# zheminzhou/PEPPAN

Hardware: AMD Instinct MI355X
Metric: gene_pairs_aligned_per_s (higher is better)
Workload: dtype int16; 1 GPU; synthgenes-v1 seed 355: 10000 genes x 1002 nt, all-vs-all (BASELINE configs[2] search stage), min_id 0.45 min_ratio...; queries_per_rank=10000, reference_genes_per_rank=10000

## Files before the change

### peppan_amd/csrc/capi.hip

```cpp
#include "common.h"
#include <chrono>
#include <time.h>
#include <algorithm>
#include <cmath>
#include <cstring>
#include <new>

int pep_fail(pep_ctx *ctx, int code, const std::string &msg)
{
    if (ctx) { ctx->n_down = 0; ctx->pin_down_used = 0; }
    if (ctx) {
        ctx->err = msg;
        ctx->n_pending = 0;
        ctx->pin_small_used = 0;
        for (auto &st : ctx->fused_state) st.dirty = true;
        for (auto &st : ctx->scan_state) st.dirty = true;
        ctx->sort_dirty = true;
        ctx->zero_clean = false;
        for (bool &f : ctx->zero_ok) f = false;
        ctx->set_clean_slots = 0;
    }
    return code;
}

int dev_reserve(pep_ctx *ctx, DevBuf &b, size_t bytes)
{
    if (bytes <= b.cap && b.p) return PEP_OK;
    if (b.p) { (void)hipFree(b.p); b.p = nullptr; b.cap = 0; }
    size_t want = std::max<size_t>(bytes + bytes / 4, 256);
    want = (want + 255) & ~(size_t)255;
    hipError_t e = hipMalloc(&b.p, want);
    if (e != hipSuccess) {
        b.p = nullptr;
        return pep_fail(ctx, PEP_ERR_HIP, std::string("hipMalloc(") + std::to_string(want) + "): " + hipGetErrorString(e));
    }
    b.cap = want;
    return PEP_OK;
}

void dev_release(DevBuf &b)
{
    if (b.p) (void)hipFree(b.p);
    b.p = nullptr;
    b.cap = 0;
}

int pin_reserve(pep_ctx *ctx, PinBuf &b, size_t bytes)
{
    if (bytes <= b.cap) return PEP_OK;
    if (b.p) (void)hipHostFree(b.p);
    b.p = nullptr; b.cap = 0;
    const size_t want = bytes + bytes / 4 + 4096;
    PEP_HIP(ctx, hipHostMalloc(reinterpret_cast<void **>(&b.p), want, hipHostMallocDefault));
    b.cap = want;
    return PEP_OK;
}

int pep_h2d(pep_ctx *ctx, void *d_dst, const void *h_src, size_t n)
{
    if (n == 0) return PEP_OK;
    if (n < ((size_t)64 << 10) || n > ((size_t)256 << 20)) {
        PEP_HIP(ctx, hipMemcpyAsync(d_dst, h_src, n, hipMemcpyHostToDevice, ctx->stream));
        return PEP_OK;
    }
    const size_t need = (n + 255) & ~(size_t)255;
    if (ctx->pin_up_used + need > ctx->pin_up.cap) {
        if (ctx->up_event_set) { PEP_HIP(ctx, pep_event_wait(ctx->up_event)); ctx->up_event_set = false; }
        ctx->pin_up_used = 0;
        if (need > ctx->pin_up.cap) PEP_TRY(pin_reserve(ctx, ctx->pin_up, std::max(need, (size_t)32 << 20)));
    }
    memcpy(ctx->pin_up.p + ctx->pin_up_used, h_src, n);
    PEP_HIP(ctx, hipMemcpyAsync(d_dst, ctx->pin_up.p + ctx->pin_up_used, n, hipMemcpyHostToDevice, ctx->stream));
    ctx->pin_up_used += need;
    if (!ctx->up_event && hipEventCreateWithFlags(&ctx->up_event, pep_wait_event_flags()) != hipSuccess) return pep_fail(ctx, PEP_ERR_HIP, "hipEventCreate failed");
    PEP_HIP(ctx, hipEventRecord(ctx->up_event, ctx->stream));
    ctx->up_event_set = true;
    return PEP_OK;
}

int pep_d2h_queue(pep_ctx *ctx, void *h_dst, const void *d_src, size_t n)
{
    if (n == 0) return PEP_OK;
    const size_t need = (n + 255) & ~(size_t)255;
    if (n < ((size_t)64 << 10) || n > ((size_t)256 << 20) || ctx->n_down >= 16) {
        PEP_HIP(ctx, hipMemcpyAsync(h_dst, d_src, n, hipMemcpyDeviceToHost, ctx->stream));
        return PEP_OK;
    }
    if (ctx->pin_down_used + need > ctx->pin_down.cap) {
        if (ctx->n_down) {
            PEP_HIP(ctx, hipMemcpyAsync(h_dst, d_src, n, hipMemcpyDeviceToHost, ctx->stream));
            return PEP_OK;
        }
        PEP_HIP(ctx, pep_stream_wait(ctx));
        PEP_TRY(pin_reserve(ctx, ctx->pin_down, std::max(need, (size_t)16 << 20)));
        ctx->pin_down_used = 0;
    }
    PEP_HIP(ctx, hipMemcpyAsync(ctx->pin_down.p + ctx->pin_down_used, d_src, n, hipMemcpyDeviceToHost, ctx->stream));
    ctx->down[ctx->n_down++] = pep_ctx::PendingDown{h_dst, ctx->pin_down_used, n};
    ctx->pin_down_used += need;
    return PEP_OK;
}

void pep_d2h_finish(pep_ctx *ctx)
{
    for (int k = 0; k < ctx->n_down; ++k) memcpy(ctx->down[k].dst, ctx->pin_down.p + ctx->down[k].off, ctx->down[k].n);
    ctx->n_down = 0;
    ctx->pin_down_used = 0;
}

void pep_timer_begin(pep_ctx *ctx, int id)
{
    if (ctx->timing_level < (id == TM_SW ? 1 : 2)) return;
    if (!ctx->tm_a[id] && (hipEventCreate(&ctx->tm_a[id]) != hipSuccess || hipEventCreate(&ctx->tm_b[id]) != hipSuccess)) { ctx->tm_a[id] = nullptr; return; }
    ctx->tm_state[id] = hipEventRecord(ctx->tm_a[id], ctx->stream) == hipSuccess ? 1 : 0;
}

void pep_timer_end(pep_ctx *ctx, int id)
{
    if (ctx->tm_state[id] == 1) ctx->tm_state[id] = hipEventRecord(ctx->tm_b[id], ctx->stream) == hipSuccess ? 2 : 0;
}

void pep_timers_resolve(pep_ctx *ctx)
{
    double match[4] = {0., 0., 0., 0.};
    double *dst[TM_COUNT] = {&ctx->stats.ms_seed, &ctx->stats.ms_total, &ctx->stats.ms_sw, &ctx->stats.ms_sw_trace, &ctx->stats.ms_trace,
                             &match[0], &match[1], &match[2], &match[3]};
    for (int id = 0; id < TM_COUNT; ++id) {
        float ms = 0.f;
        if (ctx->tm_state[id] == 2 && hipEventSynchronize(ctx->tm_b[id]) == hipSuccess && hipEventElapsedTime(&ms, ctx->tm_a[id], ctx->tm_b[id]) == hipSuccess) *dst[id] = ms;
        ctx->tm_state[id] = 0;
    }
    ctx->stats.ms_seed_match = match[0] + match[1] + match[2] + match[3];
}

int pep_zero_block(pep_ctx *ctx, int which, size_t offset, size_t bytes, void **out)
{
    PEP_TRY(dev_reserve(ctx, ctx->d_zero, PEP_ZERO_TOTAL));
    char *p = ctx->d_zero.as<char>() + offset;
    if (!ctx->zero_ok[which]) PEP_HIP(ctx, hipMemsetAsync(p, 0, bytes, ctx->stream));
    ctx->zero_ok[which] = false;
    *out = p;
    return PEP_OK;
}

int pep_read_back(pep_ctx *ctx, void *dst, const void *d_src, size_t n)
{
    const size_t n8 = (n + 7) & ~size_t(7);
    if (ctx->n_pending >= 32 || ctx->pin_small_used + n8 > ctx->pin_small.cap) PEP_TRY(pep_sync_reads(ctx));
    if (n8 > ctx->pin_small.cap) return pep_fail(ctx, PEP_ERR_INTERNAL, "pep_read_back: value larger than the pinned page");
    PEP_HIP(ctx, hipMemcpyAsync(ctx->pin_small.p + ctx->pin_small_used, d_src, n, hipMemcpyDeviceToHost, ctx->stream));
    ctx->pending[ctx->n_pending++] = pep_ctx::PendingRead{dst, ctx->pin_small_used, n};
    ctx->pin_small_used += n8;
    return PEP_OK;
}

int pep_read_back_with_upload(pep_ctx *ctx, void *dst, const void *d_src, size_t n, void *d_up_dst, const void *pinned_up_src, uint64_t n_up_words)
{
    const size_t n8 = (n + 7) & ~size_t(7);
    if (n % 4) return pep_fail(ctx, PEP_ERR_INTERNAL, "pep_read_back_with_upload: size not a multiple of 4");
    if (ctx->n_pending >= 32 || ctx->pin_small_used + n8 > ctx->pin_small.cap) PEP_TRY(pep_sync_reads(ctx));
    if (n8 > ctx->pin_small.cap) return pep_fail(ctx, PEP_ERR_INTERNAL, "pep_read_back: value larger than the pinned page");
    PEP_TRY(pep_exchange_pinned(ctx, d_up_dst, pinned_up_src, n_up_words, ctx->pin_small.p + ctx->pin_small_used, d_src, n / 4));
    ctx->pending[ctx->n_pending++] = pep_ctx::PendingRead{dst, ctx->pin_small_used, n};
    ctx->pin_small_used += n8;
    return PEP_OK;
}

static long pep_spin_us()
{
    static const long spin_us = [] { const char *e = getenv("PEPPAN_HIP_SPIN_US"); return e ? atol(e) : 1500L; }();
    return spin_us;
}

unsigned pep_wait_event_flags() { return hipEventDisableTiming; }

hipError_t pep_event_wait(hipEvent_t ev)
{
    const long spin_us = pep_spin_us();
    if (spin_us <= 0) {
        const auto t0 = std::chrono::steady_clock::now();
        do {
            for (int spin = 0; spin < 32; ++spin) {
                const hipError_t q = hipEventQuery(ev);
                if (q != hipErrorNotReady) return q;
                __builtin_ia32_pause();
            }
        } while (std::chrono::steady_clock::now() - t0 < std::chrono::microseconds(60));
        long nap_ns = 20000;
        for (;;) {
            const hipError_t q = hipEventQuery(ev);
            if (q != hipErrorNotReady) return q;
            struct timespec ts = {0, nap_ns};
            nanosleep(&ts, nullptr);
            if (nap_ns < 200000) nap_ns += nap_ns / 2;
        }
    }
    const auto t0 = std::chrono::steady_clock::now();
    for (;;) {
        for (int spin = 0; spin < 64; ++spin) {
            const hipError_t q = hipEventQuery(ev);
            if (q != hipErrorNotReady) return q;
            __builtin_ia32_pause();
        }
        if (std::chrono::steady_clock::now() - t0 > std::chrono::microseconds(spin_us)) break;
    }
    return hipEventSynchronize(ev);
}

hipError_t pep_stream_wait(pep_ctx *ctx)
{
    if (!ctx->wait_event && hipEventCreateWithFlags(&ctx->wait_event, pep_wait_event_flags()) != hipSuccess) return hipStreamSynchronize(ctx->stream);
    const hipError_t r = hipEventRecord(ctx->wait_event, ctx->stream);
    if (r != hipSuccess) return hipStreamSynchronize(ctx->stream);
    return pep_event_wait(ctx->wait_event);
}

int pep_sync_reads(pep_ctx *ctx)
{
    const hipError_t e = pep_stream_wait(ctx);
    if (e == hipSuccess)
        for (int i = 0; i < ctx->n_pending; ++i) memcpy(ctx->pending[i].dst, ctx->pin_small.p + ctx->pending[i].off, ctx->pending[i].n);
    ctx->n_pending = 0;
    ctx->pin_small_used = 0;
    if (e != hipSuccess) return pep_fail(ctx, PEP_ERR_HIP, std::string("hipStreamSynchronize: ") + hipGetErrorString(e));
    return PEP_OK;
}

void pep_drop_dev_result(pep_ctx *ctx)
{
    pep_result *r = ctx->dev_result;
    ctx->dev_result = nullptr;
    if (r && ctx->staged_result != r) r->ctx = nullptr;
}

void pep_materialise_staged(pep_ctx *ctx)
{
    pep_result *r = ctx->staged_result;
    if (!r) return;
    r->hits.assign(r->st_hits, r->st_hits + r->n_hits);
    r->cigar.assign(r->st_cigar, r->st_cigar + r->n_cigar);
    r->st_hits = nullptr; r->st_cigar = nullptr;
    if (ctx->dev_result != r) r->ctx = nullptr;
    ctx->staged_result = nullptr;
}

int pep_upload_blk2seq(pep_ctx *ctx, SeqSet &s)
{
    const uint64_t nblk = s.total / 32 + 2;
    std::vector<uint2> m(nblk, make_uint2(0u, 0u));
    for (uint32_t i = 0; i < s.n; ++i) {
        if (s.h_len[i] == 0) continue;
        const uint64_t b0 = s.h_off[i] / 32, b1 = ((uint64_t)s.h_off[i] + s.h_len[i] - 1) / 32;
        for (uint64_t b = b0; b <= b1 && b < nblk; ++b) m[b] = make_uint2(i, s.h_off[i]);
    }
    PEP_TRY(dev_reserve(ctx, s.blk2seq, nblk * sizeof(uint2)));
    PEP_HIP(ctx, hipMemcpy(s.blk2seq.p, m.data(), nblk * sizeof(uint2), hipMemcpyHostToDevice));
    return PEP_OK;
}

namespace {

const char *kBlosum62Text =
    "   A  R  N  D  C  Q  E  G  H  I  L  K  M  F  P  S  T  W  Y  V  B  Z  X  *\n"
    "A  4 -1 -2 -2  0 -1 -1  0 -2 -1 -1 -1 -1 -2 -1  1  0 -3 -2  0 -2 -1  0 -4\n"
    "R -1  5  0 -2 -3  1  0 -2  0 -3 -2  2 -1 -3 -2 -1 -1 -3 -2 -3 -1  0 -1 -4\n"
    "N -2  0  6  1 -3  0  0  0  1 -3 -3  0 -2 -3 -2  1  0 -4 -2 -3  3  0 -1 -4\n"
    "D -2 -2  1  6 -3  0  2 -1 -1 -3 -4 -1 -3 -3 -1  0 -1 -4 -3 -3  4  1 -1 -4\n"
    "C  0 -3 -3 -3  9 -3 -4 -3 -3 -1 -1 -3 -1 -2 -3 -1 -1 -2 -2 -1 -3 -3 -2 -4\n"
    "Q -1  1  0  0 -3  5  2 -2  0 -3 -2  1  0 -3 -1  0 -1 -2 -1 -2  0  3 -1 -4\n"
    "E -1  0  0  2 -4  2  5 -2  0 -3 -3  1 -2 -3 -1  0 -1 -3 -2 -2  1  4 -1 -4\n"
    "G  0 -2  0 -1 -3 -2 -2  6 -2 -4 -4 -2 -3 -3 -2  0 -2 -2 -3 -3 -1 -2 -1 -4\n"
    "H -2  0  1 -1 -3  0  0 -2  8 -3 -3 -1 -2 -1 -2 -1 -2 -2  2 -3  0  0 -1 -4\n"
    "I -1 -3 -3 -3 -1 -3 -3 -4 -3  4  2 -3  1  0 -3 -2 -1 -3 -1  3 -3 -3 -1 -4\n"
    "L -1 -2 -3 -4 -1 -2 -3 -4 -3  2  4 -2  2  0 -3 -2 -1 -2 -1  1 -4 -3 -1 -4\n"
    "K -1  2  0 -1 -3  1  1 -2 -1 -3 -2  5 -1 -3 -1  0 -1 -3 -2 -2  0  1 -1 -4\n"
    "M -1 -1 -2 -3 -1  0 -2 -3 -2  1  2 -1  5  0 -2 -1 -1 -1 -1  1 -3 -1 -1 -4\n"
    "F -2 -3 -3 -3 -2 -3 -3 -3 -1  0  0 -3  0  6 -4 -2 -2  1  3 -1 -3 -3 -1 -4\n"
    "P -1 -2 -2 -1 -3 -1 -1 -2 -2 -3 -3 -1 -2 -4  7 -1 -1 -4 -3 -2 -2 -1 -2 -4\n"
    "S  1 -1  1  0 -1  0  0  0 -1 -2 -2  0 -1 -2 -1  4  1 -3 -2 -2  0  0  0 -4\n"
    "T  0 -1  0 -1 -1 -1 -1 -2 -2 -1 -1 -1 -1 -2 -1  1  5 -2 -2  0 -1 -1  0 -4\n"
    "W -3 -3 -4 -4 -2 -2 -3 -2 -2 -3 -2 -3 -1  1 -4 -3 -2 11  2 -3 -4 -3 -2 -4\n"
    "Y -2 -2 -2 -3 -2 -1 -2 -3  2 -1 -1 -2 -1  3 -3 -2 -2  2  7 -1 -3 -2 -1 -4\n"
    "V  0 -3 -3 -3 -1 -2 -2 -3 -3  3  1 -2  1 -1 -2 -2  0 -3 -1  4 -3 -2 -1 -4\n"
    "B -2 -1  3  4 -3  0  1 -1  0 -3 -4  0 -3 -3 -2  0 -1 -4 -3 -3  4  1 -1 -4\n"
    "Z -1  0  0  1 -3  3  4 -2  0 -3 -3  1 -1 -3 -1  0 -1 -3 -2 -2  1  4 -1 -4\n"
    "X  0 -1 -1 -1 -2 -1 -1 -1 -1 -1 -1 -1 -1 -1 -2  0  0 -2 -1 -1 -1 -1 -1 -4\n"
    "* -4 -4 -4 -4 -4 -4 -4 -4 -4 -4 -4 -4 -4 -4 -4 -4 -4 -4 -4 -4 -4 -4 -4  1\n";

void parse_blosum(int8_t sub[1024])
{
    char cols[32];
    int ncol = 0;
    const char *p = kBlosum62Text;
    while (*p != '\n') { if (*p != ' ') cols[ncol++] = *p; ++p; }
    ++p;
    int m[26][26];
    bool have[26] = {false};
    for (int r = 0; r < ncol; ++r) {
        while (*p == ' ') ++p;
        const char row = *p++;
        for (int c = 0; c < ncol; ++c) {
            char *end;
            const long v = strtol(p, &end, 10);
            p = end;
            if (row >= 'A' && row <= 'Z' && cols[c] >= 'A' && cols[c] <= 'Z') { m[row - 'A'][cols[c] - 'A'] = (int)v; have[row - 'A'] = true; }
        }
        while (*p && *p != '\n') ++p;
        if (*p) ++p;
    }
    const int X = 'X' - 'A';
    for (int a = 0; a < 32; ++a)
        for (int b = 0; b < 32; ++b) {
            int v = -64;
            if (a < 26 && b < 26) v = m[have[a] ? a : X][have[b] ? b : X];
            sub[a * 32 + b] = (int8_t)v;
        }
}

int upload_sub_image(pep_ctx *ctx)
{
    std::vector<uint32_t> img(256 * PEP_TAB_REP);
    const int8_t *s = ctx->params.sub;
    for (int w = 0; w < 256; ++w) {
        const int q = w >> 3, t0 = (w & 7) * 4;
        uint32_t v = 0;
        for (int k = 0; k < 4; ++k) v |= (uint32_t)(uint8_t)s[q * 32 + t0 + k] << (8 * k);
        for (int b = 0; b < PEP_TAB_REP; ++b) img[w * PEP_TAB_REP + b] = v;
    }
    PEP_TRY(dev_reserve(ctx, ctx->sub_lds, img.size() * 4));
    PEP_HIP(ctx, hipMemcpy(ctx->sub_lds.p, img.data(), img.size() * 4, hipMemcpyHostToDevice));
    return PEP_OK;
}

int upload_nt(pep_ctx *ctx, NtSet &s, const uint8_t *nt, const uint64_t *off, uint32_t n)
{
    if (n && (!nt || !off)) return pep_fail(ctx, PEP_ERR_ARG, "null sequence buffer");
    s.n = n;
    s.h_off.assign(n + 1, 0);
    for (uint32_t i = 0; i <= n; ++i) {
        s.h_off[i] = n ? off[i] : 0;
        if (i && s.h_off[i] < s.h_off[i - 1]) return pep_fail(ctx, PEP_ERR_ARG, "offsets must be non-decreasing");
        if (i && s.h_off[i] - s.h_off[i - 1] > 0x7FFFFF00ull) return pep_fail(ctx, PEP_ERR_LIMIT, "nucleotide sequence longer than 2^31 - 256");
    }
    s.total = s.h_off[n];
    PEP_TRY(dev_reserve(ctx, s.nt, s.total + 64));
    PEP_TRY(dev_reserve(ctx, s.off, (size_t)(n + 1) * 8));
    if (s.total) PEP_TRY(pep_h2d(ctx, s.nt.p, nt, s.total));
    PEP_TRY(pep_h2d(ctx, s.off.p, s.h_off.data(), (size_t)(n + 1) * 8));
    return PEP_OK;
}

int upload_aa(pep_ctx *ctx, SeqSet &s, const uint8_t *codes, const uint64_t *off, uint32_t n, uint32_t max_n)
{
    if (n && (!codes || !off)) return pep_fail(ctx, PEP_ERR_ARG, "null sequence buffer");
    if (n > max_n) return pep_fail(ctx, PEP_ERR_LIMIT, "too many sequences");
    if (&s == &ctx->t) ctx->t_tables_lazy = false;
    if (&s == &ctx->q) ctx->q_tables_lazy = false;
    s.n = n;
    s.h_off.assign(n + 1, 0);
    s.h_len.assign(n, 0);
    uint64_t pos = PEP_END_PAD, residues = 0;
    uint32_t max_len = 0;
    for (uint32_t i = 0; i < n; ++i) {
        if (off[i + 1] < off[i]) return pep_fail(ctx, PEP_ERR_ARG, "offsets must be non-decreasing");
        const uint64_t len = off[i + 1] - off[i];
        if (len > PEP_MAX_SEQ_LEN) return pep_fail(ctx, PEP_ERR_LIMIT, "sequence longer than PEP_MAX_SEQ_LEN");
        s.h_off[i] = (uint32_t)pos;
        s.h_len[i] = (uint32_t)len;
        residues += len;
        max_len = std::max<uint32_t>(max_len, (uint32_t)len);
        pos += (len + 15) / 16 * 16 + PEP_SEQ_GAP;
        if (pos > PEP_MAX_RESIDUES) return pep_fail(ctx, PEP_ERR_LIMIT, "packed protein set exceeds 2^29 bytes");
    }
    pos += PEP_END_PAD;
    s.h_off[n] = (uint32_t)pos;
    s.total = pos; s.residues = residues; s.max_len = max_len;
    std::vector<uint8_t> img(pos, (uint8_t)PEP_PAD_CODE);
    for (uint32_t i = 0; i < n; ++i)
        for (uint32_t x = 0; x < s.h_len[i]; ++x) {
            const uint8_t c = codes[off[i] + x];
            img[s.h_off[i] + x] = c < 26 ? c : (uint8_t)23;
        }
    PEP_TRY(dev_reserve(ctx, s.res, pos + 64));
    PEP_TRY(dev_reserve(ctx, s.off, (size_t)(n + 1) * 4));
    PEP_TRY(dev_reserve(ctx, s.len, (size_t)(n + 1) * 4));
    PEP_HIP(ctx, hipMemcpy(s.res.p, img.data(), pos, hipMemcpyHostToDevice));
    PEP_HIP(ctx, hipMemcpy(s.off.p, s.h_off.data(), (size_t)(n + 1) * 4, hipMemcpyHostToDevice));
    if (n) PEP_HIP(ctx, hipMemcpy(s.len.p, s.h_len.data(), (size_t)n * 4, hipMemcpyHostToDevice));
    return pep_upload_blk2seq(ctx, s);
}

int download_aa(pep_ctx *ctx, const SeqSet &s, uint8_t *codes, uint64_t cap, uint64_t *off)
{
    if (s.residues > cap) return pep_fail(ctx, PEP_ERR_ARG, "output buffer too small");
    PEP_TRY(pep_k1_host_tables(ctx));
    std::vector<uint8_t> img(s.total);
    if (s.total) PEP_HIP(ctx, hipMemcpy(img.data(), s.res.p, s.total, hipMemcpyDeviceToHost));
    uint64_t pos = 0;
    for (uint32_t i = 0; i < s.n; ++i) {
        off[i] = pos;
        memcpy(codes + pos, img.data() + s.h_off[i], s.h_len[i]);
        pos += s.h_len[i];
    }
    off[s.n] = pos;
    return PEP_OK;
}

}

int pep_upload_codes(pep_ctx *ctx, SeqSet &s, const uint8_t *codes, const uint64_t *off, uint32_t n, uint32_t max_n) { return upload_aa(ctx, s, codes, off, n, max_n); }
int pep_upload_sub(pep_ctx *ctx) { return upload_sub_image(ctx); }

extern "C" {

int pep_version(void) { return PEP_ABI_VERSION; }

int pep_device_count(void)
{
    int n = 0;
    if (hipGetDeviceCount(&n) != hipSuccess) return 0;
    return n;
}

void pep_default_params(pep_search_params *p)
{
    memset(p, 0, sizeof(*p));
    p->gap_open = 11; p->gap_ext = 1;
    parse_blosum(p->sub);
    memset(p->reduce, 0xFF, sizeof(p->reduce));
    const char *groups = "KREDQN/C/G/H/ILV/M/F/Y/W/P/STA";
    int g = 0;
    for (const char *c = groups; *c; ++c) { if (*c == '/') ++g; else p->reduce[*c - 'A'] = (uint8_t)g; }
    p->base = g + 1;
    const char *shapes[2] = {"111101110111", "111011010010111"};
    p->n_shapes = 2;
    for (int s = 0; s < 2; ++s) {
        int w = 0;
        for (int k = 0; shapes[s][k]; ++k) if (shapes[s][k] == '1') p->offs[s][w++] = k;
        p->weight[s] = w;
    }
    p->min_id_pct = 0.; p->min_qcov_pct = 0.; p->top_k = 10; p->n_splits = 5;
    p->dbsize = 5e6; p->max_evalue = 1.;
    p->use_lds = 1;
    p->ungapped_min = 55; p->xdrop = 12; p->ext_right = 40; p->ext_left = 24; p->stage1_min = 24; p->reserved2 = 0;
    p->ka_lambda = 0.267; p->ka_k = 0.041;
}

int pep_set_sensitivity(pep_search_params *p, int level)
{
    if (!p || level < 0 || level > 1) return PEP_ERR_ARG;
    const char *shapes[4] = {"111101110111", "111011010010111", "110010011111011", "10111110011011"};
    p->n_shapes = level == 0 ? 2 : 4;
    for (int s = 0; s < 4; ++s) {
        int w = 0;
        for (int k = 0; k < 32; ++k) p->offs[s][k] = 0;
        if (s < p->n_shapes) for (int k = 0; shapes[s][k]; ++k) if (shapes[s][k] == '1') p->offs[s][w++] = k;
        p->weight[s] = w;
    }
    return PEP_OK;
}

int32_t pep_min_score_ka(uint32_t qlen, double dbsize, double max_evalue, double ka_lambda, double ka_k)
{
    const double s = log(ka_k * (double)qlen * dbsize / max_evalue) / ka_lambda;
    const int32_t r = (int32_t)ceil(s);
    return r < 1 ? 1 : r;
}

int32_t pep_min_score(uint32_t qlen, double dbsize, double max_evalue)
{
    return pep_min_score_ka(qlen, dbsize, max_evalue, 0.267, 0.041);
}

int pep_ctx_create(int device, pep_ctx **out)
{
    if (!out) return PEP_ERR_ARG;
    *out = nullptr;
    int n = 0;
    if (hipGetDeviceCount(&n) != hipSuccess || device < 0 || device >= n) return PEP_ERR_HIP;
    pep_ctx *ctx = new (std::nothrow) pep_ctx();
    if (!ctx) return PEP_ERR_INTERNAL;
    ctx->device = device;
    memset(&ctx->stats, 0, sizeof(ctx->stats));
    pep_default_params(&ctx->params);
    if (hipSetDevice(device) != hipSuccess) { delete ctx; return PEP_ERR_HIP; }
    if (hipStreamCreate(&ctx->stream) != hipSuccess) { delete ctx; return PEP_ERR_HIP; }
    if (pin_reserve(ctx, ctx->pin_small, 16384) != PEP_OK) { *out = ctx; return PEP_ERR_HIP; }
    int rc = pep_selftest_dpp(ctx);
    if (rc != PEP_OK) { *out = ctx; return rc; }
    *out = ctx;
    return PEP_OK;
}

void pep_ctx_destroy(pep_ctx *ctx)
{
    if (!ctx) return;
    (void)hipSetDevice(ctx->device);
    for (auto &b : ctx->ws) dev_release(b);
    for (int id = 0; id < TM_COUNT; ++id) { if (ctx->tm_a[id]) (void)hipEventDestroy(ctx->tm_a[id]); if (ctx->tm_b[id]) (void)hipEventDestroy(ctx->tm_b[id]); }
    pep_drop_dev_result(ctx);
    if (ctx->staged_result) {
        pep_materialise_staged(ctx);
    }
    if (ctx->pin_small.p) (void)hipHostFree(ctx->pin_small.p);
    if (ctx->pin_stage.p) (void)hipHostFree(ctx->pin_stage.p);
    if (ctx->pin_k1.p) (void)hipHostFree(ctx->pin_k1.p);
    if (ctx->pin_k1q.p) (void)hipHostFree(ctx->pin_k1q.p);
    if (ctx->pin_labels.p) (void)hipHostFree(ctx->pin_labels.p);
    if (ctx->pin_nt_match.p) (void)hipHostFree(ctx->pin_nt_match.p);
    if (ctx->k1_event) (void)hipEventDestroy(ctx->k1_event);
    if (ctx->k1q_event) (void)hipEventDestroy(ctx->k1q_event);
    if (ctx->k1_t0) (void)hipEventDestroy(ctx->k1_t0);
    if (ctx->k1_t1) (void)hipEventDestroy(ctx->k1_t1);
    if (ctx->wait_event) (void)hipEventDestroy(ctx->wait_event);
    if (ctx->up_event) (void)hipEventDestroy(ctx->up_event);
    if (ctx->pin_down.p) (void)hipHostFree(ctx->pin_down.p);
    if (ctx->pin_up.p) (void)hipHostFree(ctx->pin_up.p);
    if (ctx->pin_ms.p) (void)hipHostFree(ctx->pin_ms.p);
    DevBuf *bufs[] = {&ctx->sub_lds, &ctx->d_params, &ctx->scan_state[0].buf, &ctx->scan_state[1].buf, &ctx->fused_state[0].buf, &ctx->fused_state[1].buf, &ctx->fused_state[2].buf, &ctx->fused_state[3].buf, &ctx->d_min_score, &ctx->d_trace_mode, &ctx->d_trace_defer, &ctx->d_k1_base, &ctx->d_k1_seg, &ctx->d_k1_long, &ctx->d_k1_spec, &ctx->d_k1_tiles, &ctx->d_t_class, &ctx->d_t_subject, &ctx->d_nt_match, &ctx->q_nt.nt, &ctx->q_nt.off, &ctx->r_nt.nt, &ctx->r_nt.off,
                      &ctx->q.res, &ctx->q.off, &ctx->q.len, &ctx->t.res, &ctx->t.off, &ctx->t.len, &ctx->q.blk2seq, &ctx->t.blk2seq,
                      &ctx->sort_state, &ctx->sort_hist, &ctx->d_set, &ctx->d_zero, &ctx->d_k1_desc_q, &ctx->d_k1_desc_t, &ctx->d_self_delta, &ctx->d_self_t, &ctx->d_mail_copy,
                      &ctx->nucl_q.d_off, &ctx->nucl_q.d_len, &ctx->nucl_q.d_desc, &ctx->nucl_t.d_off, &ctx->nucl_t.d_len, &ctx->nucl_t.d_desc, &ctx->nucl_t.d_first};
    for (DevBuf *b : bufs) dev_release(*b);
    if (ctx->stream) (void)hipStreamDestroy(ctx->stream);
    delete ctx;
}

const char *pep_last_error(const pep_ctx *ctx) { return ctx ? ctx->err.c_str() : "null context"; }

int pep_set_query_nt(pep_ctx *ctx, const uint8_t *nt, const uint64_t *off, uint32_t n, int gtable)
{
    if (!ctx) return PEP_ERR_ARG;
    PEP_HIP(ctx, hipSetDevice(ctx->device));
    if (n > PEP_MAX_QUERIES) return pep_fail(ctx, PEP_ERR_LIMIT, "too many queries");
    PEP_TRY(upload_nt(ctx, ctx->q_nt, nt, off, n));
    ctx->nucl_valid = false;
    ctx->q_from_nt = true; ctx->q_gtable = gtable; ctx->q_ready = false; ctx->resid_from_nucl = false;
    return PEP_OK;
}

int pep_set_ref_nt(pep_ctx *ctx, const uint8_t *nt, const uint64_t *off, uint32_t n, int frames, int gtable)
{
    if (!ctx) return PEP_ERR_ARG;
    if (frames != 3 && frames != 6) return pep_fail(ctx, PEP_ERR_ARG, "frames must be 3 or 6");
    PEP_HIP(ctx, hipSetDevice(ctx->device));
    PEP_TRY(upload_nt(ctx, ctx->r_nt, nt, off, n));
    ctx->nucl_valid = false;
    ctx->t_from_nt = true; ctx->t_gtable = gtable; ctx->t_frames = frames; ctx->t_ready = false; ctx->k1_base_frames = 0; ctx->resid_from_nucl = false;
    ctx->group_of_seq.clear(); ctx->t_class_ready = false;
    return PEP_OK;
}

int pep_set_query_aa(pep_ctx *ctx, const uint8_t *codes, const uint64_t *off, uint32_t n)
{
    if (!ctx) return PEP_ERR_ARG;
    PEP_HIP(ctx, hipSetDevice(ctx->device));
    PEP_TRY(upload_aa(ctx, ctx->q, codes, off, n, PEP_MAX_QUERIES));
    ctx->q_meta.resize(n);
    for (uint32_t i = 0; i < n; ++i) ctx->q_meta[i] = pep_query_meta{i, 0u, ctx->q.h_len[i], 0u};
    ctx->q_from_nt = false; ctx->q_ready = true; ctx->resid_from_nucl = false;
    return PEP_OK;
}

int pep_set_ref_aa(pep_ctx *ctx, const uint8_t *codes, const uint64_t *off, uint32_t n)
{
    if (!ctx) return PEP_ERR_ARG;
    PEP_HIP(ctx, hipSetDevice(ctx->device));
    PEP_TRY(upload_aa(ctx, ctx->t, codes, off, n, PEP_MAX_TARGETS));
    ctx->t_meta.resize(n);
    for (uint32_t i = 0; i < n; ++i) ctx->t_meta[i] = pep_target_meta{i, 0u, 0u, ctx->t.h_len[i]};
    ctx->t_from_nt = false; ctx->t_ready = true; ctx->resid_from_nucl = false;
    ctx->group_of_seq.clear(); ctx->t_class_ready = false;
    return PEP_OK;
}

int pep_translate(pep_ctx *ctx, int force)
{
    if (!ctx) return PEP_ERR_ARG;
    PEP_HIP(ctx, hipSetDevice(ctx->device));
    if (!ctx->k1_t0 && (hipEventCreate(&ctx->k1_t0) != hipSuccess || hipEventCreate(&ctx->k1_t1) != hipSuccess)) { ctx->k1_t0 = ctx->k1_t1 = nullptr; }
    ctx->resid_from_nucl = false;
    const bool do_q = ctx->q_from_nt && (force || !ctx->q_ready), do_t = ctx->t_from_nt && (force || !ctx->t_ready);
    if (!do_q && !do_t) return PEP_OK;
    const bool timed = ctx->timing_level >= 2 && ctx->k1_t0;
    if (timed) (void)hipEventRecord(ctx->k1_t0, ctx->stream);
    if (do_t) PEP_TRY(pep_k1_ref(ctx, ctx->t_frames, ctx->t_gtable, 1));
    if (do_q) PEP_TRY(pep_k1_query(ctx, ctx->q_gtable, 1));
    if (do_t) { PEP_TRY(pep_k1_ref(ctx, ctx->t_frames, ctx->t_gtable, 2)); ctx->t_ready = true; }
    if (do_q) { PEP_TRY(pep_k1_query(ctx, ctx->q_gtable, 2)); ctx->q_ready = true; }
    float ms = 0.f;
    if (timed && ctx->k1_t1 && hipEventRecord(ctx->k1_t1, ctx->stream) == hipSuccess && pep_event_wait(ctx->k1_t1) == hipSuccess) (void)hipEventElapsedTime(&ms, ctx->k1_t0, ctx->k1_t1);
    ctx->stats.ms_k1 = ms;
    return PEP_OK;
}

int pep_invalidate_translation(pep_ctx *ctx)
{
    if (!ctx) return PEP_ERR_ARG;
    if (ctx->q_from_nt) ctx->q_ready = false;
    if (ctx->t_from_nt) ctx->t_ready = false;
    return PEP_OK;
}

int pep_use_nt_as_residues(pep_ctx *ctx, int strands)
{
    if (!ctx) return PEP_ERR_ARG;
    if (strands != 1 && strands != 2) return pep_fail(ctx, PEP_ERR_ARG, "strands must be 1 or 2");
    if (!ctx->q_from_nt || !ctx->t_from_nt) return pep_fail(ctx, PEP_ERR_STATE, "pep_use_nt_as_residues needs pep_set_query_nt and pep_set_ref_nt first");
    PEP_HIP(ctx, hipSetDevice(ctx->device));
    pep_materialise_staged(ctx);
    ctx->q_ready = ctx->t_ready = false;
    ctx->resid_from_nucl = false;
    ctx->t_class_ready = false;
    PEP_TRY(pep_nucl_sets(ctx, strands));
    ctx->resid_from_nucl = true;
    return PEP_OK;
}

int pep_query_count(pep_ctx *ctx, uint32_t *n, uint64_t *residues)
{
    if (!ctx || !(ctx->q_ready || ctx->resid_from_nucl)) return pep_fail(ctx, PEP_ERR_STATE, "queries not set / not translated");
    if (n) *n = ctx->q.n;
    if (residues) *residues = ctx->q.residues;
    return PEP_OK;
}

int pep_target_count(pep_ctx *ctx, uint32_t *n, uint64_t *residues)
{
    if (!ctx || !(ctx->t_ready || ctx->resid_from_nucl)) return pep_fail(ctx, PEP_ERR_STATE, "targets not set / not translated");
    if (n) *n = ctx->t.n;
    if (residues) *residues = ctx->t.residues;
    return PEP_OK;
}

int pep_get_query_meta(pep_ctx *ctx, pep_query_meta *out, uint32_t cap)
{
    if (!ctx || !(ctx->q_ready || ctx->resid_from_nucl)) return pep_fail(ctx, PEP_ERR_STATE, "queries not set / not translated");
    PEP_TRY(pep_k1_host_tables_q(ctx));
    if (cap < ctx->q_meta.size()) return pep_fail(ctx, PEP_ERR_ARG, "output buffer too small");
    if (!ctx->q_meta.empty()) memcpy(out, ctx->q_meta.data(), ctx->q_meta.size() * sizeof(pep_query_meta));
    return PEP_OK;
}

int pep_get_target_meta(pep_ctx *ctx, pep_target_meta *out, uint32_t cap)
{
    if (!ctx || !(ctx->t_ready || ctx->resid_from_nucl)) return pep_fail(ctx, PEP_ERR_STATE, "targets not set / not translated");
    PEP_TRY(pep_k1_host_tables(ctx));
    if (cap < ctx->t_meta.size()) return pep_fail(ctx, PEP_ERR_ARG, "output buffer too small");
    if (!ctx->t_meta.empty()) memcpy(out, ctx->t_meta.data(), ctx->t_meta.size() * sizeof(pep_target_meta));
    return PEP_OK;
}

int pep_get_query_aa(pep_ctx *ctx, uint8_t *codes, uint64_t cap, uint64_t *off)
{
    if (!ctx || !(ctx->q_ready || ctx->resid_from_nucl)) return pep_fail(ctx, PEP_ERR_STATE, "queries not set / not translated");
    PEP_HIP(ctx, hipSetDevice(ctx->device));
    return download_aa(ctx, ctx->q, codes, cap, off);
}

int pep_get_target_aa(pep_ctx *ctx, uint8_t *codes, uint64_t cap, uint64_t *off)
{
    if (!ctx || !(ctx->t_ready || ctx->resid_from_nucl)) return pep_fail(ctx, PEP_ERR_STATE, "targets not set / not translated");
    PEP_HIP(ctx, hipSetDevice(ctx->device));
    return download_aa(ctx, ctx->t, codes, cap, off);
}

int pep_set_target_groups(pep_ctx *ctx, const uint32_t *group, uint32_t n)
{
    if (!ctx || (n && !group)) return PEP_ERR_ARG;
    for (uint32_t i = 1; i < n; ++i)
        if (group[i] < group[i - 1]) return pep_fail(ctx, PEP_ERR_ARG, "pep_set_target_groups: groups must be contiguous and non-decreasing");
    if (ctx->group_of_seq.size() == n && (n == 0 || memcmp(ctx->group_of_seq.data(), group, (size_t)n * sizeof(uint32_t)) == 0)) return PEP_OK;
    ctx->group_of_seq.assign(group, group + n);
    ctx->t_class_ready = false;
    ctx->nucl_valid = false;
    return PEP_OK;
}

static int build_t_class(pep_ctx *ctx)
{
    ctx->t_class_ready = false;
    if (ctx->group_of_seq.empty()) return PEP_OK;
    const uint32_t n_seq = ctx->t_from_nt ? ctx->r_nt.n : ctx->t.n;
    if (ctx->group_of_seq.size() != n_seq) return pep_fail(ctx, PEP_ERR_ARG, "pep_set_target_groups: one group per reference sequence expected");
    PEP_TRY(pep_k1_host_tables(ctx));
    const uint32_t nt = ctx->t.n, ns = (uint32_t)ctx->params.n_splits;
    std::vector<uint32_t> cls(nt + 1, 0u);
    uint32_t cur = 0xFFFFFFFFu, local = 0;
    for (uint32_t t = 0; t < nt; ++t) {
        const uint32_t g = ctx->group_of_seq[ctx->t_meta[t].seq];
        if (g != cur) { cur = g; local = 0; }
        if ((uint64_t)g * ns + ns > 0xFFFFFFFFull) return pep_fail(ctx, PEP_ERR_LIMIT, "too many target groups");
        cls[t] = g * ns + local % ns;
        ++local;
    }
    PEP_TRY(dev_reserve(ctx, ctx->d_t_class, (size_t)(nt + 1) * 4));
    PEP_TRY(pep_h2d(ctx, ctx->d_t_class.p, cls.data(), (size_t)(nt + 1) * 4));
    ctx->t_class_ready = true;
    return PEP_OK;
}

int pep_search(pep_ctx *ctx, const pep_search_params *params, pep_result **out)
{
    if (!ctx || !out) return PEP_ERR_ARG;
    *out = nullptr;
    PEP_HIP(ctx, hipSetDevice(ctx->device));
    pep_materialise_staged(ctx);
    if (params) {
        if (params->n_shapes < 1 || params->n_shapes > 4 || params->base < 2 || params->top_k < 1 || params->n_splits < 1)
            return pep_fail(ctx, PEP_ERR_ARG, "invalid search parameters");
        if (params->gap_open < 0 || params->gap_open > 255 || params->gap_ext < 1 || params->gap_ext > 255)
            return pep_fail(ctx, PEP_ERR_ARG, "gap costs: 0 <= gap_open <= 255 and 1 <= gap_ext <= 255");
        for (int s = 0; s < params->n_shapes; ++s) {
            if (params->weight[s] < 1 || params->weight[s] > 32) return pep_fail(ctx, PEP_ERR_ARG, "invalid seed weight");
            if (params->offs[s][params->weight[s] - 1] > 31) return pep_fail(ctx, PEP_ERR_ARG, "seed span above 32");
            if (pow((double)params->base, params->weight[s]) > 34359738368.0) return pep_fail(ctx, PEP_ERR_ARG, "seed key does not fit 35 bits");
            if (params->base > 15 || pow((double)params->base, (params->weight[s] + 1) / 2) > 4294967295.0)
                return pep_fail(ctx, PEP_ERR_ARG, "reduced alphabet above 15 letters / half key above 32 bits");
            for (int c = 0; c < 32; ++c)
                if (params->reduce[c] != 0xFF && params->reduce[c] >= params->base) return pep_fail(ctx, PEP_ERR_ARG, "reduced letter outside the alphabet");
        }
        if (params->t_index_base < 0) return pep_fail(ctx, PEP_ERR_ARG, "t_index_base must not be negative");
        if (params->hsp_mode < 0 || params->hsp_mode > 2) return pep_fail(ctx, PEP_ERR_ARG, "hsp_mode must be 0, 1 or 2");
        if (params->stage1_min < 0 || (params->ungapped_min > 0 && params->stage1_min > params->ungapped_min))
            return pep_fail(ctx, PEP_ERR_ARG, "stage1_min must lie between 0 and ungapped_min");
        if (!(params->ka_lambda > 0.) || !(params->ka_k > 0.)) return pep_fail(ctx, PEP_ERR_ARG, "invalid Karlin-Altschul parameters");
        if (!(params->dbsize > 0.) || !(params->max_evalue > 0.)) return pep_fail(ctx, PEP_ERR_ARG, "dbsize and max_evalue must be positive");
        if (params->xdrop < 0 || params->xdrop > 48 || params->ext_right < 1 || params->ext_right > 48 || params->ext_left < 0 || params->ext_left > 48)
            return pep_fail(ctx, PEP_ERR_ARG, "invalid ungapped-extension parameters");
        for (int c = 0; c < 32; ++c)
            if (params->sub[PEP_PAD_CODE * 32 + c] > -64 || params->sub[c * 32 + PEP_PAD_CODE] > -64)
                return pep_fail(ctx, PEP_ERR_ARG, "substitution table: row and column 31 (the padding code) must be <= -64");
        if (memcmp(ctx->params.sub, params->sub, sizeof(params->sub)) != 0) ctx->sub_ready = false;
        ctx->params = *params;
    }
    ctx->k1_t_deferred = false;
    if (!ctx->resid_from_nucl) {
        const bool do_q = ctx->q_from_nt && !ctx->q_ready, do_t = ctx->t_from_nt && !ctx->t_ready;
        if ((do_q || do_t) && ctx->timing_level < 2 && ctx->group_of_seq.empty()) {
            if (do_q) PEP_TRY(pep_k1_query(ctx, ctx->q_gtable, 1));
            if (do_t) PEP_TRY(pep_k1_ref(ctx, ctx->t_frames, ctx->t_gtable, 1));
            if (do_q) { PEP_TRY(pep_k1_query(ctx, ctx->q_gtable, 2)); ctx->q_ready = true; }
            ctx->k1_t_deferred = do_t;
            ctx->stats.ms_k1 = 0.;
        } else PEP_TRY(pep_translate(ctx, 0));
        if (!ctx->q_ready || !(ctx->t_ready || ctx->k1_t_deferred)) { ctx->k1_t_deferred = false; return pep_fail(ctx, PEP_ERR_STATE, "pep_search before both sequence sets were given"); }
    }
    auto finish_targets = [](pep_ctx *c) -> int {
        if (!c->k1_t_deferred) return PEP_OK;
        c->k1_t_deferred = false;
        PEP_TRY(pep_k1_ref(c, c->t_frames, c->t_gtable, 2));
        c->t_ready = true;
        c->stats.target_residues = c->t.residues;
        return PEP_OK;
    };
    if (!ctx->sub_ready) { const int rc0 = upload_sub_image(ctx); if (rc0 != PEP_OK) { ctx->k1_t_deferred = false; return rc0; } ctx->sub_ready = true; }
    { const int rc0 = build_t_class(ctx); if (rc0 != PEP_OK) { ctx->k1_t_deferred = false; return rc0; } }

    pep_result *res = new (std::nothrow) pep_result();
    if (!res) { ctx->k1_t_deferred = false; return pep_fail(ctx, PEP_ERR_INTERNAL, "out of host memory"); }
    res->ctx = ctx;
    const double ms_k1 = ctx->stats.ms_k1;
    memset(&ctx->stats, 0, sizeof(ctx->stats));
    ctx->stats.ms_k1 = ms_k1;
    ctx->stats.query_residues = ctx->q.residues;
    ctx->stats.target_residues = ctx->t.residues;

    for (int id = 0; id < TM_COUNT; ++id) ctx->tm_state[id] = 0;
    pep_timer_begin(ctx, TM_SEED); pep_timer_begin(ctx, TM_TOTAL);
    uint64_t *d_cands = nullptr, n_cands = 0;
    auto prepare_thresholds = [](pep_ctx *c) -> int {
        PEP_TRY(dev_reserve(c, c->d_min_score, (size_t)(c->q.n + 1) * 4));
        PEP_TRY(pin_reserve(c, c->pin_ms, (size_t)(c->q.n + 1) * 4));
        int32_t *ms = reinterpret_cast<int32_t *>(c->pin_ms.p);
        uint32_t memo_len[1024];
        int32_t memo_val[1024];
        for (int i = 0; i < 1024; ++i) memo_len[i] = 0xFFFFFFFFu;
        for (uint32_t i = 0; i < c->q.n; ++i) {
            const uint32_t L = c->q.h_len[i], slot = L & 1023u;
            if (memo_len[slot] != L) {
                memo_len[slot] = L;
                memo_val[slot] = pep_min_score_ka(L, c->params.dbsize, c->params.max_evalue, c->params.ka_lambda, c->params.ka_k);
            }
            ms[i] = memo_val[slot];
        }
        c->upload.d_dst = c->d_min_score.p; c->upload.pinned_src = c->pin_ms.p; c->upload.n_words = c->q.n;
        return PEP_OK;
    };
    int rc = pep_find_candidates(ctx, &d_cands, &n_cands, prepare_thresholds, finish_targets);
    if (rc == PEP_OK && ctx->k1_t_deferred) rc = finish_targets(ctx);
    ctx->k1_t_deferred = false;
    pep_timer_end(ctx, TM_SEED);
    if (rc == PEP_OK) rc = pep_extend(ctx, d_cands, n_cands, nullptr, res, true);
    const bool grouped = rc == PEP_OK && ctx->grp_nodes != 0;
    if (grouped)
        rc = ctx->ext.pending ? pep_k10_queue(ctx, ctx->ext.n_bound, reinterpret_cast<const pep_hit *>(ctx->ext.d_hits), ctx->ext.d_n_hits)
                              : pep_k10_queue(ctx, res->n_hits, res->d_hits);
    const bool counted = rc == PEP_OK && ctx->want_nt_match;
    if (counted)
        rc = ctx->ext.pending ? pep_k7_hits_queue(ctx, ctx->ext.n_bound, reinterpret_cast<const pep_hit *>(ctx->ext.d_hits), reinterpret_cast<const uint32_t *>(ctx->ext.d_cig), ctx->ext.d_n_hits)
                              : pep_k7_hits_queue(ctx, res->n_hits, res->d_hits, res->d_cigar);
    pep_timer_end(ctx, TM_TOTAL);
    const hipError_t se = pep_stream_wait(ctx);
    if (rc == PEP_OK && se != hipSuccess) rc = pep_fail(ctx, PEP_ERR_HIP, std::string("stream sync: ") + hipGetErrorString(se));
    if (rc == PEP_OK) rc = pep_extend_finish(ctx);
    ctx->ext.pending = false;
    if (rc != PEP_OK) { delete res; return rc; }
    pep_timers_resolve(ctx);
    if (grouped) {
        const uint32_t *lab = reinterpret_cast<const uint32_t *>(ctx->pin_labels.p);
        res->labels.assign(lab, lab + ctx->grp_nodes);
    }
    if (counted && res->n_hits) {
        const uint32_t *cnt = reinterpret_cast<const uint32_t *>(ctx->pin_nt_match.p);
        res->nt_match.assign(cnt, cnt + res->n_hits);
    }
    res->stats = ctx->stats;
    ctx->dev_result = res->d_hits ? res : nullptr;
    if (res->st_hits || res->st_cigar) ctx->staged_result = res;
    else if (!res->d_hits) res->ctx = nullptr;
    *out = res;
    return PEP_OK;
}

int pep_set_nt_match(pep_ctx *ctx, int on)
{
    if (!ctx || (on != 0 && on != 1)) return PEP_ERR_ARG;
    ctx->want_nt_match = on != 0;
    return PEP_OK;
}

int pep_result_nt_match(const pep_result *r, const uint32_t **nt_match)
{
    if (!r || !nt_match) return PEP_ERR_ARG;
    *nt_match = (r->n_hits && r->nt_match.size() == r->n_hits) ? r->nt_match.data() : nullptr;
    return PEP_OK;
}

int pep_set_timing(pep_ctx *ctx, int level)
{
    if (!ctx || level < 0 || level > 2) return PEP_ERR_ARG;
    ctx->timing_level = level;
    return PEP_OK;
}

int pep_set_grouping(pep_ctx *ctx, uint32_t n_nodes, uint32_t q_base, const uint32_t *node_of_target, uint64_t n_targets)
{
    if (!ctx || (n_nodes && n_targets && !node_of_target)) return PEP_ERR_ARG;
    PEP_HIP(ctx, hipSetDevice(ctx->device));
    return pep_k10_set_grouping(ctx, n_nodes, q_base, node_of_target, n_targets);
}

int pep_result_labels(const pep_result *r, uint32_t *label, uint32_t n_nodes)
{
    if (!r || (n_nodes && !label)) return PEP_ERR_ARG;
    if (r->labels.size() != n_nodes) return PEP_ERR_STATE;
    if (n_nodes) memcpy(label, r->labels.data(), (size_t)n_nodes * 4);
    return PEP_OK;
}

int pep_set_result_mode(pep_ctx *ctx, int on_device)
{
    if (!ctx) return PEP_ERR_ARG;
    ctx->device_results = on_device != 0;
    return PEP_OK;
}

static int pep_fetch_result(const pep_result *cr)
{
    pep_result *r = const_cast<pep_result *>(cr);
    if (r->st_hits || r->n_hits == 0 || !r->hits.empty()) return PEP_OK;
    pep_ctx *ctx = r->ctx;
    if (!ctx || ctx->dev_result != r) return PEP_ERR_STATE;
    PEP_HIP(ctx, hipSetDevice(ctx->device));
    r->hits.resize(r->n_hits);
    r->cigar.resize(r->n_cigar);
    PEP_HIP(ctx, hipMemcpyAsync(r->hits.data(), r->d_hits, r->n_hits * sizeof(pep_hit), hipMemcpyDeviceToHost, ctx->stream));
    if (r->n_cigar) PEP_HIP(ctx, hipMemcpyAsync(r->cigar.data(), r->d_cigar, r->n_cigar * 4, hipMemcpyDeviceToHost, ctx->stream));
    PEP_HIP(ctx, hipStreamSynchronize(ctx->stream));
    return PEP_OK;
}

int pep_result_size(const pep_result *r, uint64_t *n_hits, uint64_t *n_cigar)
{
    if (!r) return PEP_ERR_ARG;
    if (n_hits) *n_hits = r->n_hits;
    if (n_cigar) *n_cigar = r->n_cigar;
    return PEP_OK;
}

int pep_result_copy(const pep_result *r, pep_hit *hits, uint32_t *cigar)
{
    if (!r) return PEP_ERR_ARG;
    PEP_TRY(pep_fetch_result(r));
    const pep_hit *h = r->st_hits ? r->st_hits : r->hits.data();
    const uint32_t *c = r->st_cigar ? r->st_cigar : r->cigar.data();
    if (hits && r->n_hits) memcpy(hits, h, r->n_hits * sizeof(pep_hit));
    if (cigar && r->n_cigar) memcpy(cigar, c, r->n_cigar * sizeof(uint32_t));
    return PEP_OK;
}

int pep_result_data(const pep_result *r, const pep_hit **hits, const uint32_t **cigar)
{
    if (!r) return PEP_ERR_ARG;
    PEP_TRY(pep_fetch_result(r));
    if (hits) *hits = r->st_hits ? r->st_hits : r->hits.data();
    if (cigar) *cigar = r->st_cigar ? r->st_cigar : r->cigar.data();
    return PEP_OK;
}

int pep_result_stats(const pep_result *r, pep_stats *stats)
{
    if (!r || !stats) return PEP_ERR_ARG;
    *stats = r->stats;
    return PEP_OK;
}

void pep_result_free(pep_result *r)
{
    if (r && r->ctx && r->ctx->staged_result == r) r->ctx->staged_result = nullptr;
    if (r && r->ctx && r->ctx->dev_result == r) r->ctx->dev_result = nullptr;
    delete r;
}

int pep_result_device(const pep_result *r, const pep_hit **d_hits, const uint32_t **d_cigar)
{
    if (!r) return PEP_ERR_ARG;
    const bool live = r->ctx && r->ctx->dev_result == r;
    if (d_hits) *d_hits = live ? r->d_hits : nullptr;
    if (d_cigar) *d_cigar = live ? r->d_cigar : nullptr;
    return live ? PEP_OK : PEP_ERR_STATE;
}

int pep_components_of_result(pep_ctx *ctx, const pep_result *r, uint32_t n_nodes, uint32_t q_base, const uint32_t *node_of_target, uint64_t n_targets, uint32_t *label)
{
    if (!ctx || !r || (n_nodes && !label) || (n_targets && !node_of_target)) return PEP_ERR_ARG;
    PEP_HIP(ctx, hipSetDevice(ctx->device));
    if (r->ctx == ctx && ctx->dev_result == r && n_targets >= ctx->t.n)
        return pep_k10_components_dev(ctx, n_nodes, r->n_hits, r->d_hits, q_base, node_of_target, n_targets, label);
    PEP_TRY(pep_fetch_result(r));
    const pep_hit *h = r->st_hits ? r->st_hits : r->hits.data();
    return pep_components_of_hits(ctx, n_nodes, r->n_hits, h, q_base, node_of_target, n_targets, label);
}

int pep_merge_hits(uint64_t n, const pep_hit *hits, const uint32_t *cigar, uint64_t n_cigar, int32_t top_k, int32_t n_splits,
                   pep_hit *out_hits, uint32_t *out_cigar, uint64_t *n_out, uint64_t *n_cigar_out)
{
    if (!n_out || !n_cigar_out || top_k < 1 || n_splits < 1 || (n && (!hits || !out_hits)) || (n_cigar && (!cigar || !out_cigar))) return PEP_ERR_ARG;
    *n_out = 0; *n_cigar_out = 0;
    if (n == 0) return PEP_OK;
    if (n > 0xFFFFFFFFull) return PEP_ERR_LIMIT;
    uint32_t q_hi = 0;
    for (uint64_t i = 0; i < n; ++i) {
        if (hits[i].cigar_off + hits[i].cigar_runs > n_cigar) return PEP_ERR_ARG;
        q_hi = std::max(q_hi, hits[i].q);
    }
    auto by_t = [&](uint32_t a, uint32_t b) {
        const pep_hit &x = hits[a], &y = hits[b];
        if (x.t != y.t) return x.t < y.t;
        return x.bin < y.bin;
    };
    std::vector<uint32_t> order((size_t)n), first;
    if ((uint64_t)q_hi <= 64 * n + (1u << 20)) {
        first.assign((size_t)q_hi + 2, 0);
        for (uint64_t i = 0; i < n; ++i) ++first[hits[i].q + 1];
        for (size_t q = 1; q < first.size(); ++q) first[q] += first[q - 1];
        std::vector<uint32_t> at(first.begin(), first.end() - 1);
        for (uint64_t i = 0; i < n; ++i) order[at[hits[i].q]++] = (uint32_t)i;
    } else {
        for (uint64_t i = 0; i < n; ++i) order[i] = (uint32_t)i;
        std::stable_sort(order.begin(), order.end(), [&](uint32_t a, uint32_t b) { return hits[a].q < hits[b].q; });
    }
    std::vector<uint32_t> grp, count((size_t)n_splits);
    std::vector<uint8_t> drop;
    uint64_t no = 0, nc = 0;
    for (uint64_t a = 0; a < n;) {
        uint64_t b = a + 1;
        bool sorted = true;
        const uint32_t q = hits[order[a]].q;
        while (b < n && hits[order[b]].q == q) { sorted = sorted && !by_t(order[b], order[b - 1]); ++b; }
        if (!sorted) std::sort(order.begin() + a, order.begin() + b, by_t);
        bool over = false;
        if (b - a > (uint64_t)top_k) {
            std::fill(count.begin(), count.end(), 0u);
            for (uint64_t k = a; k < b; ++k) over = (++count[hits[order[k]].t % (uint32_t)n_splits] > (uint32_t)top_k) || over;
        }
        if (over) {
            if (drop.empty()) drop.assign((size_t)n, 0);
            for (int32_t sp = 0; sp < n_splits; ++sp) {
                if (count[sp] <= (uint32_t)top_k) continue;
                grp.clear();
                for (uint64_t k = a; k < b; ++k)
                    if ((int32_t)(hits[order[k]].t % (uint32_t)n_splits) == sp) grp.push_back(order[k]);
                std::sort(grp.begin(), grp.end(), [&](uint32_t u, uint32_t v) {
                    const pep_hit &x = hits[u], &y = hits[v];
                    if (x.score != y.score) return x.score > y.score;
                    return by_t(u, v);
                });
                for (size_t k = (size_t)top_k; k < grp.size(); ++k) drop[grp[k]] = 1;
            }
        }
        for (uint64_t k = a; k < b; ++k) {
            const uint32_t i = order[k];
            if (over && drop[i]) continue;
            pep_hit h = hits[i];
            if (h.cigar_runs) memcpy(out_cigar + nc, cigar + h.cigar_off, (size_t)h.cigar_runs * sizeof(uint32_t));
            h.cigar_off = nc;
            nc += h.cigar_runs;
            out_hits[no++] = h;
        }
        a = b;
    }
    *n_out = no; *n_cigar_out = nc;
    return PEP_OK;
}

int pep_rescore_nt(pep_ctx *ctx, uint64_t n, const pep_nt_hit *hits, const uint32_t *cigar, uint64_t n_cigar, int64_t *out)
{
    if (!ctx || (n && (!hits || !cigar || !out))) return PEP_ERR_ARG;
    PEP_HIP(ctx, hipSetDevice(ctx->device));
    return pep_k7_rescore(ctx, n, hits, cigar, n_cigar, out);
}

int pep_components(pep_ctx *ctx, uint32_t n_nodes, uint64_t n_edges, const uint32_t *a, const uint32_t *b, uint32_t *label)
{
    if (!ctx || (n_nodes && !label) || (n_edges && (!a || !b))) return PEP_ERR_ARG;
    PEP_HIP(ctx, hipSetDevice(ctx->device));
    return pep_k10_components(ctx, n_nodes, n_edges, a, b, label);
}

int pep_components_of_hits(pep_ctx *ctx, uint32_t n_nodes, uint64_t n_hits, const pep_hit *hits, uint32_t q_base,
                           const uint32_t *node_of_target, uint64_t n_targets, uint32_t *label)
{
    if (!ctx || (n_nodes && !label) || (n_hits && (!hits || !node_of_target))) return PEP_ERR_ARG;
    PEP_HIP(ctx, hipSetDevice(ctx->device));
    std::vector<uint32_t> a(n_hits + 1), b(n_hits + 1);
    for (uint64_t h = 0; h < n_hits; ++h) {
        if (hits[h].t >= n_targets) return pep_fail(ctx, PEP_ERR_ARG, "pep_components_of_hits: target index out of range");
        a[h] = hits[h].q + q_base;
        b[h] = node_of_target[hits[h].t];
    }
    return pep_k10_components(ctx, n_nodes, n_hits, a.data(), b.data(), label);
}

int pep_linclust(pep_ctx *ctx, const uint8_t *codes, const uint64_t *off, uint32_t n, int base, int k, int m, double min_id, double min_cov,
                 uint32_t *rep, uint64_t *stats)
{
    if (!ctx || (n && (!codes || !off || !rep))) return PEP_ERR_ARG;
    PEP_HIP(ctx, hipSetDevice(ctx->device));
    for (uint32_t i = 0; i < n; ++i)
        if (off[i + 1] < off[i]) return pep_fail(ctx, PEP_ERR_ARG, "offsets must be non-decreasing");
    return pep_k9_linclust(ctx, codes, off, n, base, k, m, min_id, min_cov, rep, stats);
}

int pep_overlaps(pep_ctx *ctx, uint64_t n, const int32_t *contig, const int64_t *start, const int64_t *end, const int64_t *row_id,
                 double ovl_l, double ovl_p, int64_t *out, uint64_t cap, uint64_t *n_pairs)
{
    if (!ctx || !n_pairs || (n && (!contig || !start || !end || !row_id)) || (cap && !out)) return PEP_ERR_ARG;
    PEP_HIP(ctx, hipSetDevice(ctx->device));
    return pep_k11_overlaps(ctx, n, contig, start, end, row_id, ovl_l, ovl_p, out, cap, n_pairs);
}

int pep_alleles(pep_ctx *ctx, const uint8_t *nt, const uint64_t *nt_off, uint32_t n_contigs, uint64_t n_rows, const pep_locus *rows,
                const uint32_t *cigar, uint64_t n_cigar, uint32_t n_groups, const uint64_t *grp_off, const uint32_t *grp_qlen, int gtable,
                int64_t *in_frame, int64_t *orf, uint8_t *packed, uint64_t packed_cap)
{
    if (!ctx || !nt_off || (n_rows && (!rows || !cigar || !in_frame || !orf)) || (n_groups && (!grp_off || !grp_qlen || !packed))) return PEP_ERR_ARG;
    PEP_HIP(ctx, hipSetDevice(ctx->device));
    for (uint32_t i = 0; i < n_contigs; ++i)
        if (nt_off[i + 1] < nt_off[i]) return pep_fail(ctx, PEP_ERR_ARG, "offsets must be non-decreasing");
    if (n_contigs && nt_off[n_contigs] && !nt) return PEP_ERR_ARG;
    return pep_k12_alleles(ctx, nt, nt_off, n_contigs, n_rows, rows, cigar, n_cigar, n_groups, grp_off, grp_qlen, gtable, in_frame, orf, packed, packed_cap);
}

int pep_allele_diff(pep_ctx *ctx, const uint8_t *packed, const uint64_t *row_off, const uint32_t *row_len, uint64_t n_rows,
                    uint32_t n_groups, const uint64_t *grp_off, const uint32_t *grp_rows, const uint8_t *grp_mode,
                    int32_t *out, const uint64_t *out_off, uint64_t out_cap)
{
    if (!ctx) return PEP_ERR_ARG;
    if (!row_off || (n_rows && !row_len) || (n_groups && (!grp_off || !grp_mode || !out_off)) || (out_cap && !out))
        return pep_fail(ctx, PEP_ERR_ARG, "pep_allele_diff: null table");
    if (n_groups && grp_off[n_groups] && !grp_rows) return pep_fail(ctx, PEP_ERR_ARG, "pep_allele_diff: null table");
    if (n_rows && row_off[n_rows] && !packed) return pep_fail(ctx, PEP_ERR_ARG, "pep_allele_diff: null table");
    PEP_HIP(ctx, hipSetDevice(ctx->device));
    return pep_k15_allele_diff(ctx, packed, row_off, row_len, n_rows, n_groups, grp_off, grp_rows, grp_mode, out, out_off, out_cap);
}

int pep_allele_diff_times(const pep_ctx *ctx, double *ms_planes, double *ms_pairs, double *ms_copy_back)
{
    if (!ctx || !ms_planes || !ms_pairs || !ms_copy_back) return PEP_ERR_ARG;
    *ms_planes = ctx->k15_ms[0];
    *ms_pairs = ctx->k15_ms[1];
    *ms_copy_back = ctx->k15_ms[2];
    return PEP_OK;
}

int pep_sha1(pep_ctx *ctx, const uint8_t *bytes, const uint64_t *off, uint32_t n, uint8_t *digest)
{
    if (!ctx || (n && (!off || !digest))) return PEP_ERR_ARG;
    PEP_HIP(ctx, hipSetDevice(ctx->device));
    for (uint32_t i = 0; i < n; ++i)
        if (off[i + 1] < off[i]) return pep_fail(ctx, PEP_ERR_ARG, "offsets must be non-decreasing");
    if (n && off[n] && !bytes) return PEP_ERR_ARG;
    return pep_k13_sha1(ctx, bytes, off, n, digest);
}

int pep_dedup(pep_ctx *ctx, uint32_t n, const uint32_t *len, const uint8_t *digest, uint32_t *rep)
{
    if (!ctx || (n && (!len || !digest || !rep))) return PEP_ERR_ARG;
    if (n >= 0x7FFFFFFFu) return pep_fail(ctx, PEP_ERR_LIMIT, "pep_dedup: at most 2^31 - 2 genes");
    PEP_HIP(ctx, hipSetDevice(ctx->device));
    return pep_k13_dedup(ctx, n, len, digest, rep);
}

}
```

### peppan_amd/csrc/common.h

```cpp
#pragma once
#include <hip/hip_runtime.h>
#include <stdint.h>
#include <stddef.h>
#include <string>
#include <vector>
#include "../../include/peppan_hip.h"

#define PEP_WAVE 64
#define PEP_TAB_REP 16

#define PEP_HIP(ctx, expr)                                                                            \
    do {                                                                                              \
        hipError_t _e = (expr);                                                                       \
        if (_e != hipSuccess) {                                                                       \
            return pep_fail((ctx), PEP_ERR_HIP, std::string(#expr) + ": " + hipGetErrorString(_e));   \
        }                                                                                             \
    } while (0)

#define PEP_TRY(expr)                  \
    do {                               \
        int _rc = (expr);              \
        if (_rc != PEP_OK) return _rc; \
    } while (0)

struct DevBuf {
    void *p = nullptr;
    size_t cap = 0;
    template <class T> T *as() const { return reinterpret_cast<T *>(p); }
};

#define PEP_PAD_CODE 31
#define PEP_SEQ_GAP 16
#define PEP_END_PAD 64
struct SeqSet {
    uint32_t n = 0;
    uint64_t total = 0;
    uint64_t residues = 0;
    uint32_t max_len = 0;
    DevBuf res;
    DevBuf off;
    DevBuf len;
    DevBuf blk2seq;
    std::vector<uint32_t> h_off, h_len;
};

struct NtSet {
    uint32_t n = 0;
    uint64_t total = 0;
    DevBuf nt;
    DevBuf off;
    std::vector<uint64_t> h_off;
};

struct PinBuf {
    uint8_t *p = nullptr;
    size_t cap = 0;
};

struct pep_result;

struct PackDesc {
    uint32_t seq;
    uint32_t frame;
    uint32_t aa_off;
    uint32_t len;
};
struct NuclDesc { uint32_t seq, rev; };

struct pep_ctx {
    int device = 0;
    hipStream_t stream = nullptr;
    PinBuf pin_small;
    size_t pin_small_used = 0;
    struct PendingRead { void *dst; size_t off, n; } pending[32];
    int n_pending = 0;
    PinBuf pin_k1, pin_k1q;
    DevBuf d_k1_desc_q, d_k1_desc_t;
    DevBuf d_self_delta, d_self_t;
    uint32_t self_first_n = 0;
    const uint32_t *self_first = nullptr;
    uint32_t self_first_cnt = 0;
    int self_exact_len = 0;
    hipEvent_t k1_event = nullptr;
    hipEvent_t k1q_event = nullptr;
    bool k1q_event_set = false;
    bool k1_t_deferred = false;
    hipEvent_t wait_event = nullptr;
    hipEvent_t k1_t0 = nullptr, k1_t1 = nullptr;
    uint32_t k1_desc_cap = 0;
    bool t_tables_lazy = false, q_tables_lazy = false;
    PinBuf pin_up;
    size_t pin_up_used = 0;
    hipEvent_t up_event = nullptr;
    bool up_event_set = false;
    PinBuf pin_down;
    size_t pin_down_used = 0;
    struct PendingDown { void *dst; size_t off, n; } down[16];
    int n_down = 0;
    PinBuf pin_stage;
    PinBuf pin_ms;
    pep_result *staged_result = nullptr;
    std::string err;
    pep_search_params params;
    NtSet q_nt, r_nt;
    SeqSet q, t;
    std::vector<pep_query_meta> q_meta;
    std::vector<pep_target_meta> t_meta;
    bool q_from_nt = false, t_from_nt = false;
    bool q_ready = false, t_ready = false, sub_ready = false, codon_ready = false;
    bool resid_from_nucl = false;
    int q_gtable = 11, t_gtable = 11, t_frames = 6;
    DevBuf d_k1_base;
    std::vector<uint64_t> k1_base;
    uint64_t k1_upper = 0;
    int k1_base_frames = 0;
    DevBuf d_k1_seg, d_k1_long, d_k1_spec, d_k1_tiles;
    uint32_t k1_n_seg = 0, k1_n_long = 0, k1_n_tiles = 0;
    struct NuclSide {
        uint32_t n = 0, max_len = 0;
        uint64_t total = 0, residues = 0;
        std::vector<uint32_t> h_off, h_len;
        std::vector<pep_query_meta> q_meta;
        std::vector<pep_target_meta> t_meta;
        DevBuf d_off, d_len, d_desc;
        DevBuf d_first;
        uint32_t n_first = 0;
    } nucl_q, nucl_t;
    bool nucl_valid = false;
    int nucl_strands = 0;
    DevBuf d_min_score;
    DevBuf d_trace_defer;
    DevBuf d_trace_mode;
    std::vector<uint32_t> group_of_seq;
    DevBuf d_t_class;
    DevBuf d_t_subject;
    bool t_class_ready = false;
    DevBuf ws[24];
    DevBuf sub_lds;
    DevBuf d_params;
    int8_t d_params_host[1024] = {};
    bool d_params_valid = false;
    hipEvent_t tm_a[12] = {}, tm_b[12] = {};
    int tm_state[12] = {};
    int timing_level = 0;
    PinBuf pin_labels;
    uint64_t trace_swept = 0;
    struct ScanState { DevBuf buf; uint32_t epoch = 0, ticket_base = 0; bool dirty = false; };
    ScanState fused_state[4];
    ScanState scan_state[2];
    DevBuf sort_state, sort_hist;
    uint32_t sort_epoch = 0, sort_ticket_base = 0;
    bool sort_dirty = false;
    DevBuf d_set;
    uint64_t set_clean_slots = 0;
    DevBuf uf_nodes;
    std::vector<uint32_t> uf_nodes_host;
    struct { bool pending = false; pep_result *res = nullptr; const void *d_hits = nullptr, *d_cig = nullptr; const uint32_t *d_n_hits = nullptr; uint64_t n_bound = 0; bool parent_ready = false; } ext;
    struct { void *d_dst = nullptr; const void *pinned_src = nullptr; uint64_t n_words = 0; } upload;
    bool want_nt_match = false;
    DevBuf d_nt_match;
    PinBuf pin_nt_match;
    uint32_t grp_nodes = 0, grp_q_base = 0;
    bool device_results = false;
    pep_result *dev_result = nullptr;
    DevBuf d_zero;
    bool zero_clean = false;
    DevBuf d_mail_copy;
    bool zero_ok[4] = {false, false, false, false};
    double k15_ms[3] = {0., 0., 0.};
    pep_stats stats;
};

struct pep_result {
    pep_ctx *ctx = nullptr;
    std::vector<pep_hit> hits;
    std::vector<uint32_t> cigar;
    const pep_hit *st_hits = nullptr;
    const uint32_t *st_cigar = nullptr;
    uint64_t n_hits = 0, n_cigar = 0;
    const pep_hit *d_hits = nullptr;
    const uint32_t *d_cigar = nullptr;
    pep_stats stats;
    std::vector<uint32_t> labels;
    std::vector<uint32_t> nt_match;
};

hipError_t pep_event_wait(hipEvent_t ev);
unsigned pep_wait_event_flags();

struct EventTimer {
    hipEvent_t a = nullptr, b = nullptr;
    hipStream_t st;
    explicit EventTimer(hipStream_t s) : st(s)
    {
        if (hipEventCreate(&a) != hipSuccess) a = nullptr;
        if (hipEventCreate(&b) != hipSuccess) b = nullptr;
        if (a) (void)hipEventRecord(a, st);
    }
    float stop()
    {
        float ms = 0.f;
        if (a && b && hipEventRecord(b, st) == hipSuccess && pep_event_wait(b) == hipSuccess) (void)hipEventElapsedTime(&ms, a, b);
        return ms;
    }
    ~EventTimer()
    {
        if (a) (void)hipEventDestroy(a);
        if (b) (void)hipEventDestroy(b);
    }
    EventTimer(const EventTimer &) = delete;
    EventTimer &operator=(const EventTimer &) = delete;
};

enum PepTimer { TM_SEED = 0, TM_TOTAL, TM_SW, TM_SW_TRACE, TM_TRACE, TM_MATCH0, TM_MATCH1, TM_MATCH2, TM_MATCH3, TM_COUNT };
void pep_timer_begin(pep_ctx *ctx, int id);
void pep_timer_end(pep_ctx *ctx, int id);
void pep_timers_resolve(pep_ctx *ctx);

int pep_fail(pep_ctx *ctx, int code, const std::string &msg);
int pep_read_back(pep_ctx *ctx, void *dst, const void *d_src, size_t n);
int pep_sync_reads(pep_ctx *ctx);
hipError_t pep_stream_wait(pep_ctx *ctx);
hipError_t pep_event_wait(hipEvent_t ev);
int pin_reserve(pep_ctx *ctx, PinBuf &b, size_t bytes);
int pep_h2d(pep_ctx *ctx, void *d_dst, const void *h_src, size_t n);
int pep_d2h_queue(pep_ctx *ctx, void *h_dst, const void *d_src, size_t n);
void pep_d2h_finish(pep_ctx *ctx);
void pep_materialise_staged(pep_ctx *ctx);
void pep_drop_dev_result(pep_ctx *ctx);
int dev_reserve(pep_ctx *ctx, DevBuf &b, size_t bytes);
void dev_release(DevBuf &b);

#define PEP_ZERO_SEED 0
#define PEP_SORT_TOP_BITS 10
#define PEP_SORT_TOP_CAP 4096
#define PEP_ZERO_TOP (PEP_ZERO_SEED + 64)
#define PEP_ZERO_SHAPE (PEP_ZERO_TOP + 4096)
#define PEP_ZERO_COARSE (PEP_ZERO_SHAPE + 64)
#define PEP_ZERO_SORT (PEP_ZERO_COARSE + 4 * 8192 * 4)
#define PEP_ZERO_SW_BYTES (64 + 2 * 1024 * 4)
#define PEP_ZERO_SW_SCORE (PEP_ZERO_SORT + 8 * 2048 * 4)
#define PEP_ZERO_SW_TRACE (PEP_ZERO_SW_SCORE + PEP_ZERO_SW_BYTES)
#define PEP_ZERO_SELECT (PEP_ZERO_SW_TRACE + PEP_ZERO_SW_BYTES)
#define PEP_ZERO_TILES (PEP_ZERO_SELECT + 256)
#define PEP_ZERO_TOTAL (PEP_ZERO_TILES + 4 * 8 * 128)
enum { PEP_ZC_SW_SCORE = 0, PEP_ZC_SW_TRACE, PEP_ZC_SELECT, PEP_ZC_SORT };
int pep_zero_block(pep_ctx *ctx, int which, size_t offset, size_t bytes, void **out);

int pep_scan_u32(pep_ctx *ctx, const uint32_t *d_in, uint32_t *d_out, uint64_t n, DevBuf &tmp, uint32_t *d_total = nullptr);
int pep_scan_u64(pep_ctx *ctx, const uint64_t *d_in, uint64_t *d_out, uint64_t n, DevBuf &tmp, uint64_t *d_total = nullptr);
int pep_copy_from_pinned(pep_ctx *ctx, void *d_dst, const void *pinned_src, uint64_t n_words);
int pep_exchange_pinned(pep_ctx *ctx, void *d_up_dst, const void *pinned_up_src, uint64_t n_up_words, void *pinned_down_dst, const void *d_down_src, uint64_t n_down_words);
int pep_read_back_with_upload(pep_ctx *ctx, void *dst, const void *d_src, size_t n, void *d_up_dst, const void *pinned_up_src, uint64_t n_up_words);
struct pep_key_unpack { int on, tb, bb; uint32_t bin_min; };
int pep_sort_u64(pep_ctx *ctx, uint64_t *d_keys, uint64_t *d_tmp, const uint32_t *d_n, uint64_t n_bound, int bits, uint32_t *d_hist_zeroed,
                 const pep_key_unpack *unpack);
int pep_sort_u64_two_level(pep_ctx *ctx, uint64_t *d_keys, uint64_t *d_tmp, uint64_t n, int bits, const uint32_t *d_top_hist, const pep_key_unpack *unpack);
int pep_k1_query(pep_ctx *ctx, int gtable, int phase = 0);
int pep_k1_ref(pep_ctx *ctx, int frames, int gtable, int phase = 0);
int pep_k1_host_tables(pep_ctx *ctx);
int pep_k1_host_tables_q(pep_ctx *ctx);
int pep_nucl_sets(pep_ctx *ctx, int strands);
int pep_find_candidates(pep_ctx *ctx, uint64_t **d_cands, uint64_t *n_cands, int (*before_sync)(pep_ctx *) = nullptr, int (*need_targets)(pep_ctx *) = nullptr);
int pep_upload_sub_table(pep_ctx *ctx);
int pep_sw_run(pep_ctx *ctx, const uint64_t *d_cands, uint64_t n, bool trace, const int32_t *d_known = nullptr, const int32_t *d_end_lane = nullptr, const int32_t *d_skip_mode = nullptr,
               const uint32_t *d_n = nullptr, uint64_t dir_blocks_bound = 0, unsigned long long **d_hdr = nullptr);
int pep_extend(pep_ctx *ctx, const uint64_t *d_cands, uint64_t n_cands, const int32_t *h_min_score, pep_result *res, bool defer = false);
int pep_extend_finish(pep_ctx *ctx);
int pep_selftest_dpp(pep_ctx *ctx);
int pep_k7_rescore(pep_ctx *ctx, uint64_t n, const pep_nt_hit *h_hits, const uint32_t *h_cigar, uint64_t n_cigar, int64_t *h_out);
int pep_k10_components(pep_ctx *ctx, uint32_t n_nodes, uint64_t n_edges, const uint32_t *h_a, const uint32_t *h_b, uint32_t *h_label);
int pep_k10_components_dev(pep_ctx *ctx, uint32_t n_nodes, uint64_t n_hits, const pep_hit *d_hits, uint32_t q_base, const uint32_t *h_node_of_target,
                           uint64_t n_targets, uint32_t *h_label);

int pep_k7_hits_queue(pep_ctx *ctx, uint64_t n_hits, const pep_hit *d_hits, const uint32_t *d_cigar, const uint32_t *d_n_hits = nullptr);
int pep_k10_queue(pep_ctx *ctx, uint64_t n_hits, const pep_hit *d_hits, const uint32_t *d_n_hits = nullptr);
int pep_k10_set_grouping(pep_ctx *ctx, uint32_t n_nodes, uint32_t q_base, const uint32_t *h_node_of_target, uint64_t n_targets);

int pep_k11_overlaps(pep_ctx *ctx, uint64_t n, const int32_t *h_contig, const int64_t *h_start, const int64_t *h_end, const int64_t *h_rid,
                     double ovl_l, double ovl_p, int64_t *h_out, uint64_t cap, uint64_t *n_pairs);
int pep_k12_alleles(pep_ctx *ctx, const uint8_t *h_nt, const uint64_t *h_nt_off, uint32_t n_contigs, uint64_t n, const pep_locus *h_rows,
                    const uint32_t *h_cigar, uint64_t n_cigar, uint32_t n_groups, const uint64_t *h_grp_off, const uint32_t *h_grp_qlen,
                    int gtable, int64_t *h_in_frame, int64_t *h_orf, uint8_t *h_packed, uint64_t packed_cap);
int pep_k15_allele_diff(pep_ctx *ctx, const uint8_t *h_packed, const uint64_t *h_row_off, const uint32_t *h_row_len, uint64_t n_rows,
                        uint32_t n_groups, const uint64_t *h_grp_off, const uint32_t *h_grp_rows, const uint8_t *h_grp_mode,
                        int32_t *h_out, const uint64_t *h_out_off, uint64_t out_cap);
int pep_k13_sha1(pep_ctx *ctx, const uint8_t *h_bytes, const uint64_t *h_off, uint32_t n, uint8_t *h_digest);
int pep_k13_dedup(pep_ctx *ctx, uint32_t n, const uint32_t *h_len, const uint8_t *h_digest, uint32_t *h_rep);
int pep_k14_pair_support(pep_ctx *ctx, uint64_t n_rows, const pep_support_row *h_rows, const uint32_t *h_cigar, uint64_t n_cigar, uint64_t n_groups,
                         const uint64_t *h_grp_off, const uint32_t *h_qlen, const uint32_t *h_rlen, const pep_support_limits *lim, int32_t *h_value);
int pep_k9_linclust(pep_ctx *ctx, const uint8_t *h_res, const uint64_t *h_off, uint32_t n, int base, int k, int m, double min_id, double min_cov,
                    uint32_t *h_rep, uint64_t *h_stats);

static inline uint64_t ceil_div(uint64_t a, uint64_t b) { return (a + b - 1) / b; }
int pep_upload_blk2seq(pep_ctx *ctx, SeqSet &s);
#define PEP_SELF_NONE 0xFFFFFFFFu
#define PEP_SELF_NO_DELTA ((int32_t)0x80808080)
int pep_self_map(pep_ctx *ctx, int *on);
int pep_upload_codes(pep_ctx *ctx, SeqSet &s, const uint8_t *codes, const uint64_t *off, uint32_t n, uint32_t max_n);
int pep_upload_sub(pep_ctx *ctx);
```

### peppan_amd/csrc/lookback.h

```cpp
#pragma once
#include "common.h"

constexpr uint64_t LB_SUM = 1, LB_PREFIX = 2;

__device__ __forceinline__ uint32_t lb_take_tile(uint64_t *state, uint32_t ticket_base, uint32_t *s_tile)
{
    if (threadIdx.x == 0) *s_tile = atomicAdd(reinterpret_cast<uint32_t *>(state), 1u) - ticket_base;
    __syncthreads();
    return *s_tile;
}

template <int VB>
__device__ __forceinline__ uint64_t lb_tile_prefix(uint64_t *status, uint32_t tile, uint64_t tot, uint64_t epoch, int lane)
{
    constexpr uint64_t VMASK = (1ull << VB) - 1;
    uint64_t prefix = 0;
    if (tile > 0) {
        if (lane == 0) __hip_atomic_store(&status[tile], (epoch << (VB + 2)) | (LB_SUM << VB) | (tot & VMASK), __ATOMIC_RELAXED, __HIP_MEMORY_SCOPE_AGENT);
        for (int64_t hi = (int64_t)tile - 1; hi >= 0; hi -= 64) {
            const int64_t idx = hi - lane;
            uint64_t w = (epoch << (VB + 2)) | (LB_PREFIX << VB);
            if (idx >= 0)
                do { w = __hip_atomic_load(&status[idx], __ATOMIC_RELAXED, __HIP_MEMORY_SCOPE_AGENT); } while ((w >> (VB + 2)) != epoch);
            const uint64_t is_prefix = __ballot(((w >> VB) & 3u) == LB_PREFIX);
            const int stop = is_prefix ? __ffsll((unsigned long long)is_prefix) - 1 : 63;
            uint64_t part = lane <= stop ? (w & VMASK) : 0ull;
#pragma unroll
            for (int d = 32; d > 0; d >>= 1) part += __shfl_xor(part, d, 64);
            prefix += part;
            if (is_prefix) break;
        }
    }
    if (lane == 0) __hip_atomic_store(&status[tile], (epoch << (VB + 2)) | (LB_PREFIX << VB) | ((prefix + tot) & VMASK), __ATOMIC_RELAXED, __HIP_MEMORY_SCOPE_AGENT);
    return prefix;
}

template <class T>
__device__ __forceinline__ T block_excl_scan_256(T v, T *total, T *lds)
{
    const int lane = threadIdx.x & 63, wave = threadIdx.x >> 6;
    T inc = v;
#pragma unroll
    for (int d = 1; d < 64; d <<= 1) { const T o = __shfl_up(inc, d, 64); if (lane >= d) inc += o; }
    if (lane == 63) lds[wave] = inc;
    __syncthreads();
    T base = 0, tot = 0;
#pragma unroll
    for (int w = 0; w < 4; ++w) { const T s = lds[w]; if (w < wave) base += s; tot += s; }
    __syncthreads();
    *total = tot;
    return base + inc - v;
}

int pep_lookback_begin(pep_ctx *ctx, pep_ctx::ScanState &S, uint64_t n_tiles, uint32_t epoch_mask, uint64_t **state, uint32_t *ticket_base, uint64_t *epoch);
```

### peppan_amd/csrc/scan.hip

```cpp
#include "common.h"
#include "lookback.h"

namespace {

constexpr int SCAN_THREADS = 256;
constexpr int SCAN_ITEMS = 8;
constexpr int SCAN_TILE = SCAN_THREADS * SCAN_ITEMS;

template <class T>
__device__ __forceinline__ T wave_incl_scan(T v, int lane)
{
#pragma unroll
    for (int d = 1; d < 64; d <<= 1) {
        T o = __shfl_up(v, d, 64);
        if (lane >= d) v += o;
    }
    return v;
}

template <class T>
__device__ __forceinline__ T block_excl_scan(T v, T *total, T *lds )
{
    const int lane = threadIdx.x & 63, wave = threadIdx.x >> 6;
    T inc = wave_incl_scan(v, lane);
    if (lane == 63) lds[wave] = inc;
    __syncthreads();
    T base = 0, tot = 0;
#pragma unroll
    for (int w = 0; w < SCAN_THREADS / 64; ++w) {
        T s = lds[w];
        if (w < wave) base += s;
        tot += s;
    }
    __syncthreads();
    *total = tot;
    return base + inc - v;
}

template <class T>
__global__ __launch_bounds__(SCAN_THREADS) void scan_reduce(const T *__restrict__ in, T *__restrict__ partial, uint64_t n)
{
    __shared__ T lds[4];
    const uint64_t base = (uint64_t)blockIdx.x * SCAN_TILE;
    T s = 0;
#pragma unroll
    for (int k = 0; k < SCAN_ITEMS; ++k) {
        uint64_t i = base + (uint64_t)k * SCAN_THREADS + threadIdx.x;
        if (i < n) s += in[i];
    }
    T tot;
    block_excl_scan(s, &tot, lds);
    if (threadIdx.x == 0) partial[blockIdx.x] = tot;
}

template <class T>
__global__ __launch_bounds__(SCAN_THREADS) void scan_partials(T *partial, uint64_t nb)
{
    __shared__ T lds[4];
    T carry = 0;
    for (uint64_t b0 = 0; b0 < nb; b0 += SCAN_THREADS) {
        uint64_t i = b0 + threadIdx.x;
        T v = i < nb ? partial[i] : 0, tot;
        T ex = block_excl_scan(v, &tot, lds);
        if (i < nb) partial[i] = carry + ex;
        carry += tot;
    }
    if (threadIdx.x == 0) partial[nb] = carry;
}

template <class T>
__global__ __launch_bounds__(SCAN_THREADS) void scan_apply(const T *in, T *out, const T *__restrict__ partial,
                                                           uint64_t n, uint64_t nb)
{
    __shared__ T lds[4];
    const uint64_t base = (uint64_t)blockIdx.x * SCAN_TILE + (uint64_t)threadIdx.x * SCAN_ITEMS;
    T v[SCAN_ITEMS], s = 0;
#pragma unroll
    for (int k = 0; k < SCAN_ITEMS; ++k) {
        v[k] = (base + k < n) ? in[base + k] : 0;
        s += v[k];
    }
    T tot;
    T ex = block_excl_scan(s, &tot, lds) + partial[blockIdx.x];
#pragma unroll
    for (int k = 0; k < SCAN_ITEMS; ++k) {
        if (base + k < n) out[base + k] = ex;
        ex += v[k];
    }
    if (blockIdx.x == 0 && threadIdx.x == 0) out[n] = partial[nb];
}

constexpr uint64_t FLAG_SUM = 1, FLAG_PREFIX = 2;

template <class T> struct ScanWord;
template <> struct ScanWord<uint32_t> { static constexpr int VB = 32; static constexpr uint32_t EPOCH_MASK = (1u << 30) - 1; };
template <> struct ScanWord<uint64_t> { static constexpr int VB = 48; static constexpr uint32_t EPOCH_MASK = (1u << 14) - 1; };

template <class T>
__global__ __launch_bounds__(SCAN_THREADS) void scan_lookback(const T *in, T *out, uint64_t n, uint32_t nb, uint64_t *state, uint32_t ticket_base, uint64_t epoch,
                                                              T *total_out)
{
    constexpr int VB = ScanWord<T>::VB;
    constexpr uint64_t VMASK = (1ull << VB) - 1;
    __shared__ T lds[4];
    __shared__ uint32_t s_tile;
    __shared__ T s_prefix;
    if (threadIdx.x == 0) s_tile = atomicAdd(reinterpret_cast<uint32_t *>(state), 1u) - ticket_base;
    __syncthreads();
    const uint32_t tile = s_tile;
    uint64_t *status = state + 1;
    const uint64_t base = (uint64_t)tile * SCAN_TILE + (uint64_t)threadIdx.x * SCAN_ITEMS;
    T v[SCAN_ITEMS], s = 0;
#pragma unroll
    for (int k = 0; k < SCAN_ITEMS; ++k) {
        v[k] = (base + k < n) ? in[base + k] : 0;
        s += v[k];
    }
    T tot;
    T ex = block_excl_scan(s, &tot, lds);
    if (threadIdx.x < 64) {
        const int lane = threadIdx.x;
        T prefix = 0;
        if (tile > 0) {
            if (lane == 0) __hip_atomic_store(&status[tile], (epoch << (VB + 2)) | (FLAG_SUM << VB) | ((uint64_t)tot & VMASK), __ATOMIC_RELAXED, __HIP_MEMORY_SCOPE_AGENT);
            for (int64_t hi = (int64_t)tile - 1; hi >= 0; hi -= 64) {
                const int64_t idx = hi - lane;
                uint64_t w = (epoch << (VB + 2)) | (FLAG_PREFIX << VB);
                if (idx >= 0)
                    do { w = __hip_atomic_load(&status[idx], __ATOMIC_RELAXED, __HIP_MEMORY_SCOPE_AGENT); } while ((w >> (VB + 2)) != epoch);
                const uint64_t is_prefix = __ballot(((w >> VB) & 3u) == FLAG_PREFIX);
                const int stop = is_prefix ? __ffsll((unsigned long long)is_prefix) - 1 : 63;
                T part = lane <= stop ? (T)(w & VMASK) : (T)0;
#pragma unroll
                for (int d = 32; d > 0; d >>= 1) part += __shfl_xor(part, d, 64);
                prefix += part;
                if (is_prefix) break;
            }
        }
        if (lane == 0) {
            __hip_atomic_store(&status[tile], (epoch << (VB + 2)) | (FLAG_PREFIX << VB) | ((uint64_t)(prefix + tot) & VMASK), __ATOMIC_RELAXED, __HIP_MEMORY_SCOPE_AGENT);
            s_prefix = prefix;
        }
    }
    __syncthreads();
    ex += s_prefix;
#pragma unroll
    for (int k = 0; k < SCAN_ITEMS; ++k) {
        if (base + k < n) out[base + k] = ex;
        ex += v[k];
    }
    if (tile == nb - 1 && threadIdx.x == SCAN_THREADS - 1) { out[n] = ex; if (total_out) *total_out = ex; }
}

template <class T>
int scan_onepass(pep_ctx *ctx, const T *d_in, T *d_out, uint64_t n, T *d_total)
{
    const uint64_t nb = ceil_div(n, SCAN_TILE);
    pep_ctx::ScanState &S = ctx->scan_state[sizeof(T) == 8];
    bool clear = false;
    if ((nb + 1) * sizeof(uint64_t) > S.buf.cap) {
        PEP_TRY(dev_reserve(ctx, S.buf, (nb + 1) * sizeof(uint64_t) * 2));
        clear = true;
    }
    if (S.dirty) { clear = true; S.dirty = false; }
    S.epoch = (S.epoch + 1) & ScanWord<T>::EPOCH_MASK;
    if (S.epoch == 0) { clear = true; S.epoch = 1; }
    if (clear) {
        PEP_HIP(ctx, hipMemsetAsync(S.buf.p, 0, S.buf.cap, ctx->stream));
        S.ticket_base = 0;
    }
    hipLaunchKernelGGL(scan_lookback<T>, dim3((unsigned)nb), dim3(SCAN_THREADS), 0, ctx->stream, d_in, d_out, n, (uint32_t)nb, S.buf.as<uint64_t>(), S.ticket_base,
                       (uint64_t)S.epoch, d_total);
    S.ticket_base += (uint32_t)nb;
    PEP_HIP(ctx, hipGetLastError());
    return PEP_OK;
}

template <class T>
int scan_impl(pep_ctx *ctx, const T *d_in, T *d_out, uint64_t n, DevBuf &tmp, T *d_total)
{
    if (n == 0) {
        PEP_HIP(ctx, hipMemsetAsync(d_out, 0, sizeof(T), ctx->stream));
        if (d_total) PEP_HIP(ctx, hipMemsetAsync(d_total, 0, sizeof(T), ctx->stream));
        return PEP_OK;
    }
    const uint64_t nb = ceil_div(n, SCAN_TILE);
    PEP_TRY(dev_reserve(ctx, tmp, (nb + 1) * sizeof(T)));
    T *partial = tmp.as<T>();
    hipLaunchKernelGGL(scan_reduce<T>, dim3((unsigned)nb), dim3(SCAN_THREADS), 0, ctx->stream, d_in, partial, n);
    hipLaunchKernelGGL(scan_partials<T>, dim3(1), dim3(SCAN_THREADS), 0, ctx->stream, partial, nb);
    hipLaunchKernelGGL(scan_apply<T>, dim3((unsigned)nb), dim3(SCAN_THREADS), 0, ctx->stream, d_in, d_out, (const T *)partial, n, nb);
    if (d_total) PEP_HIP(ctx, hipMemcpyAsync(d_total, d_out + n, sizeof(T), hipMemcpyDeviceToDevice, ctx->stream));
    PEP_HIP(ctx, hipGetLastError());
    return PEP_OK;
}

}

int pep_scan_u32(pep_ctx *ctx, const uint32_t *d_in, uint32_t *d_out, uint64_t n, DevBuf &tmp, uint32_t *d_total)
{
    if (n == 0 || n >= (1ull << 40)) return scan_impl<uint32_t>(ctx, d_in, d_out, n, tmp, d_total);
    return scan_onepass<uint32_t>(ctx, d_in, d_out, n, d_total);
}

int pep_scan_u64(pep_ctx *ctx, const uint64_t *d_in, uint64_t *d_out, uint64_t n, DevBuf &tmp, uint64_t *d_total)
{
    if (n == 0 || n >= (1ull << 40)) return scan_impl<uint64_t>(ctx, d_in, d_out, n, tmp, d_total);
    return scan_onepass<uint64_t>(ctx, d_in, d_out, n, d_total);
}

namespace {
__global__ __launch_bounds__(256) void copy_words(uint32_t *__restrict__ dst, const uint32_t *__restrict__ src, uint64_t n)
{
    for (uint64_t i = (uint64_t)blockIdx.x * 256 + threadIdx.x; i < n; i += (uint64_t)gridDim.x * 256) dst[i] = src[i];
}
}

namespace {
__global__ __launch_bounds__(256) void exchange_words(uint32_t *__restrict__ up_dst, const uint32_t *__restrict__ up_src, uint64_t n_up,
                                                      uint32_t *__restrict__ down_dst, const uint32_t *__restrict__ down_src, uint64_t n_down)
{
    const uint64_t t0 = (uint64_t)blockIdx.x * 256 + threadIdx.x, stride = (uint64_t)gridDim.x * 256;
    for (uint64_t i = t0; i < n_up; i += stride) up_dst[i] = up_src[i];
    for (uint64_t i = t0; i < n_down; i += stride) down_dst[i] = down_src[i];
}
}

int pep_exchange_pinned(pep_ctx *ctx, void *d_up_dst, const void *pinned_up_src, uint64_t n_up_words, void *pinned_down_dst, const void *d_down_src, uint64_t n_down_words)
{
    if (n_up_words + n_down_words == 0) return PEP_OK;
    hipLaunchKernelGGL(exchange_words, dim3((unsigned)std::min<uint64_t>(ceil_div(std::max(n_up_words, n_down_words), 256), 1024)), dim3(256), 0, ctx->stream,
                       reinterpret_cast<uint32_t *>(d_up_dst), reinterpret_cast<const uint32_t *>(pinned_up_src), n_up_words,
                       reinterpret_cast<uint32_t *>(pinned_down_dst), reinterpret_cast<const uint32_t *>(d_down_src), n_down_words);
    PEP_HIP(ctx, hipGetLastError());
    return PEP_OK;
}

int pep_copy_from_pinned(pep_ctx *ctx, void *d_dst, const void *pinned_src, uint64_t n_words)
{
    if (n_words == 0) return PEP_OK;
    hipLaunchKernelGGL(copy_words, dim3((unsigned)std::min<uint64_t>(ceil_div(n_words, 256), 1024)), dim3(256), 0, ctx->stream, reinterpret_cast<uint32_t *>(d_dst),
                       reinterpret_cast<const uint32_t *>(pinned_src), n_words);
    PEP_HIP(ctx, hipGetLastError());
    return PEP_OK;
}

int pep_lookback_begin(pep_ctx *ctx, pep_ctx::ScanState &S, uint64_t n_tiles, uint32_t epoch_mask, uint64_t **state, uint32_t *ticket_base, uint64_t *epoch)
{
    bool clear = false;
    if ((n_tiles + 1) * sizeof(uint64_t) > S.buf.cap) {
        PEP_TRY(dev_reserve(ctx, S.buf, (n_tiles + 1) * sizeof(uint64_t) * 2));
        clear = true;
    }
    if (S.dirty) { clear = true; S.dirty = false; }
    S.epoch = (S.epoch + 1) & epoch_mask;
    if (S.epoch == 0) { clear = true; S.epoch = 1; }
    if (clear) {
        PEP_HIP(ctx, hipMemsetAsync(S.buf.p, 0, S.buf.cap, ctx->stream));
        S.ticket_base = 0;
    }
    *state = S.buf.as<uint64_t>();
    *ticket_base = S.ticket_base;
    *epoch = S.epoch;
    S.ticket_base += (uint32_t)n_tiles;
    return PEP_OK;
}
```

### peppan_amd/csrc/translate.hip

```cpp
#include "common.h"
#include "lookback.h"
#include <algorithm>

namespace {

__constant__ uint8_t c_codon[2][64];

__device__ __forceinline__ int base2(uint8_t ch)
{
    const uint32_t u = ch & 0xDFu;
    const int code = (int)(((u >> 1) ^ (u >> 2)) & 3u);
    if (u == ((0x54474341u >> (code * 8)) & 0xFFu)) return code;
    return ch == '-' ? -2 : -1;
}

__device__ __forceinline__ void nt4(uint32_t w, bool rev, uint32_t &pk, uint32_t &bad)
{
    const uint32_t u = w & 0xDFDFDFDFu;
    uint32_t code = ((u >> 1) ^ (u >> 2)) & 0x03030303u;
    const uint32_t diff = u ^ __builtin_amdgcn_perm(0u, 0x54474341u, code);
    const uint32_t nz = ((((diff & 0x7F7F7F7Fu) + 0x7F7F7F7Fu) | diff) >> 7) & 0x01010101u;
    if (rev) code ^= 0x03030303u;
    pk = (code * 0x40100401u) >> 24;
    bad = (nz * 0x08040201u) >> 24;
}

__device__ __forceinline__ int translate_at(const uint8_t *__restrict__ nt, int L, int frame, int aa, int tab, bool *is_gap)
{
    int b[3];
    const int p0 = (frame <= 3 ? frame - 1 : frame - 4) + 3 * aa;
#pragma unroll
    for (int k = 0; k < 3; ++k) {
        const int p = p0 + k;
        int v = -1;
        if (p < L) {
            if (frame <= 3) v = base2(nt[p]);
            else { v = base2(nt[L - 1 - p]); if (v >= 0) v = 3 - v; }
        }
        b[k] = v;
    }
    const bool gap = (b[0] == -2) | (b[1] == -2) | (b[2] == -2);
    if (is_gap) *is_gap = gap;
    if (gap || (b[0] | b[1] | b[2]) < 0) return 23;
    return c_codon[tab][(b[0] << 4) | (b[1] << 2) | b[2]];
}

__device__ __forceinline__ int64_t frame_len(int64_t L, int frame)
{
    const int64_t rem = L - (frame <= 3 ? frame - 1 : frame - 4);
    return rem > 0 ? (rem + 2) / 3 : 0;
}

struct K1Summary {
    unsigned long long residues, total;
    uint32_t n, max_len;
    uint32_t pad[2];
};
static_assert(sizeof(K1Summary) == 2 * 16, "the summary takes two descriptor slots");


struct K1Src { uint64_t off; uint32_t L, pad; };
static_assert(sizeof(K1Src) == sizeof(PackDesc), "source records lie behind the descriptors, in slots of the same size");
__host__ __device__ __forceinline__ K1Src *k1_src_of(const PackDesc *desc, uint32_t cap) { return reinterpret_cast<K1Src *>(const_cast<PackDesc *>(desc) + cap + 3); }

__device__ __forceinline__ uint32_t padded_len(uint32_t len) { return (len + 15u) / 16u * 16u + PEP_SEQ_GAP; }

__global__ __launch_bounds__(256) void k1_query_frames(const uint8_t *__restrict__ nt, const uint64_t *__restrict__ off, uint32_t n, int tab,
                                                       PackDesc *__restrict__ desc, uint32_t *__restrict__ padded, uint32_t *__restrict__ len_out, uint32_t *__restrict__ n_out,
                                                       K1Summary *__restrict__ sum, uint32_t *__restrict__ pin_len, K1Src *__restrict__ src_of)
{
    const int lane = threadIdx.x & 63;
    const uint32_t g = blockIdx.x * 4 + (threadIdx.x >> 6);
    if (blockIdx.x == 0 && threadIdx.x == 0) { *n_out = n; sum->residues = 0ull; sum->max_len = 0u; }
    if (g >= n) return;
    const uint64_t o = off[g];
    const uint8_t *s = nt + o;
    const int L = (int)(off[g + 1] - o);
    __shared__ uint32_t stage_all[4][392];
    uint32_t *stage = stage_all[threadIdx.x >> 6];
    const unsigned long long stop_codon = __ballot(c_codon[tab][lane] == 23);
    const int na1 = (int)frame_len(L, 1), na2 = (int)frame_len(L, 2), na3 = (int)frame_len(L, 3);
    uint32_t x1 = 0, x2 = 0, x3 = 0;
    for (int c0 = 0; c0 + 1 < na1; c0 += 512) {
        const int lo = 3 * c0;
        const uintptr_t A = reinterpret_cast<uintptr_t>(s + lo);
        const int shift = (int)(A & 3u);
        const uint32_t *al = reinterpret_cast<const uint32_t *>(A - shift);
        const int n_dw = (min(1538, L - lo) + shift + 3) >> 2;
        for (int x = lane; x < n_dw; x += 64) stage[x] = al[x];
        __builtin_amdgcn_fence(__ATOMIC_RELEASE, "workgroup");
        __builtin_amdgcn_wave_barrier();
        __builtin_amdgcn_fence(__ATOMIC_ACQUIRE, "workgroup");
        uint32_t raw[8];
#pragma unroll
        for (int k = 0; k < 8; ++k) raw[k] = stage[6 * lane + k];
        unsigned long long codes = 0;
        uint32_t bad = 0, gap = 0;
#pragma unroll
        for (int k = 0; k < 7; ++k) {
            const uint32_t w = __builtin_amdgcn_alignbyte(raw[k + 1], raw[k], (uint32_t)shift);
            uint32_t pk, bd;
            nt4(w, false, pk, bd);
            const uint32_t g = w ^ 0x2D2D2D2Du;
            const uint32_t is_gap = (~((((g & 0x7F7F7F7Fu) + 0x7F7F7F7Fu) | g)) >> 7) & 0x01010101u;
            codes |= (unsigned long long)pk << (48 - 8 * k);
            bad |= bd << (24 - 4 * k);
            gap |= ((is_gap * 0x08040201u) >> 24) << (24 - 4 * k);
        }
        const int nv = min(max(L - (lo + 24 * lane), 0), 28);
        bad |= (1u << (28 - nv)) - 1u;
        gap &= ~((1u << (28 - nv)) - 1u);
        const int lim[3] = {na1, na2, na3};
        uint32_t *cnt[3] = {&x1, &x2, &x3};
#pragma unroll
        for (int h = 0; h < 8; ++h) {
            const int a = c0 + 8 * lane + h;
#pragma unroll
            for (int f = 0; f < 3; ++f) {
                const int j = 3 * h + f;
                const uint32_t idx = (uint32_t)(codes >> (50 - 2 * j)) & 63u;
                const uint32_t b3 = (bad >> (25 - j)) & 7u, g3 = (gap >> (25 - j)) & 7u;
                const bool stop = g3 == 0u && (b3 != 0u || ((stop_codon >> idx) & 1ull));
                *cnt[f] += (a + 1 < lim[f] && stop) ? 1u : 0u;
            }
        }
        __builtin_amdgcn_wave_barrier();
    }
    for (int d = 32; d > 0; d >>= 1) { x1 += __shfl_xor(x1, d, 64); x2 += __shfl_xor(x2, d, 64); x3 += __shfl_xor(x3, d, 64); }
    uint32_t best_cnt = x1, best_f = 1, best_len = (uint32_t)na1;
    if (x2 < best_cnt) { best_cnt = x2; best_f = 2; best_len = (uint32_t)na2; }
    if (x3 < best_cnt) { best_cnt = x3; best_f = 3; best_len = (uint32_t)na3; }
    if (lane == 0) {
        desc[g] = PackDesc{g, best_f, 0u, best_len};
        src_of[g] = K1Src{o, (uint32_t)L, 0u};
        padded[g] = padded_len(best_len);
        len_out[g] = best_len;
        pin_len[g] = best_len;
    }
}

__device__ __forceinline__ int64_t chunk_end(const uint8_t *s, int64_t L, int f, int tab, int64_t na, int64_t c0, int lane)
{
    if (na + 1 - c0 < 1001) return na;
    int64_t x0 = c0 + 1000;
    for (;;) {
        const int64_t a = x0 + lane;
        bool isx = false;
        if (a < na) { bool gap; isx = (translate_at(s, (int)L, f, (int)a, tab, &gap) == 23) && !gap; }
        else if (a == na) isx = true;
        const unsigned long long m = __ballot(isx);
        if (m) return x0 + (int64_t)__ffsll((long long)m) - 1;
        x0 += 64;
    }
}

constexpr int64_t K1_LONG = 98304;
struct K1Seg { uint32_t w, seg; };
constexpr uint32_t K1_FILL_FROM = 128;
static_assert((int64_t)K1_FILL_FROM * 1001 > K1_LONG, "a frame that leaves its descriptors to k1_ref_desc_fill is a long one");
struct K1Long { uint32_t w, pad; uint64_t mask_off; };

__device__ __forceinline__ bool stop_at(const uint8_t *__restrict__ nt, int L, int frame, int aa, unsigned long long stop_codons)
{
    int b[3];
    const int p0 = (frame <= 3 ? frame - 1 : frame - 4) + 3 * aa;
#pragma unroll
    for (int k = 0; k < 3; ++k) {
        const int p = p0 + k;
        int v = -1;
        if (p < L) {
            if (frame <= 3) v = base2(nt[p]);
            else { v = base2(nt[L - 1 - p]); if (v >= 0) v = 3 - v; }
        }
        b[k] = v;
    }
    if ((b[0] == -2) | (b[1] == -2) | (b[2] == -2)) return false;
    if ((b[0] | b[1] | b[2]) < 0) return true;
    return (stop_codons >> ((b[0] << 4) | (b[1] << 2) | b[2])) & 1ull;
}

__global__ __launch_bounds__(256) void k1_stop_mask(const uint8_t *__restrict__ nt, const uint64_t *__restrict__ off, int n_frames, int tab, const K1Seg *__restrict__ tiles,
                                                    uint32_t n_tiles, const K1Long *__restrict__ longs, const uint32_t *__restrict__ long_of_w, unsigned long long *__restrict__ mask)
{
    const int lane = threadIdx.x & 63;
    const uint32_t x = blockIdx.x * 4 + (threadIdx.x >> 6);
    if (x >= n_tiles) return;
    const K1Seg tl = tiles[x];
    const uint32_t g = tl.w / (uint32_t)n_frames;
    const int f = (int)(tl.w % (uint32_t)n_frames) + 1;
    const uint8_t *s = nt + off[g];
    const int64_t L = (int64_t)(off[g + 1] - off[g]);
    const int64_t na = frame_len(L, f);
    unsigned long long *out = mask + longs[long_of_w[tl.w]].mask_off;
    const int64_t n_words = (na + 1 + 63) >> 6;
    const unsigned long long stop_codons = __ballot(c_codon[tab][lane] == 23);
    for (int64_t wd = (int64_t)tl.seg * 64; wd < (int64_t)(tl.seg + 1) * 64 && wd < n_words; wd += 4) {
        bool isx[4];
#pragma unroll
        for (int u = 0; u < 4; ++u) {
            const int64_t a = (wd + u) * 64 + lane;
            isx[u] = a < na ? stop_at(s, (int)L, f, (int)a, stop_codons) : a == na;
        }
#pragma unroll
        for (int u = 0; u < 4; ++u) {
            const unsigned long long m = __ballot(isx[u]);
            if (lane == 0 && wd + u < n_words) out[wd + u] = m;
        }
    }
}

__global__ __launch_bounds__(256) void k1_ref_chunks_mask(const uint64_t *__restrict__ off, int n_frames, const K1Long *__restrict__ longs, uint32_t n_long,
                                                          const unsigned long long *__restrict__ mask, const uint64_t *__restrict__ chunk_base,
                                                          uint32_t *__restrict__ chunk_cnt, uint32_t *__restrict__ chunk_off, uint32_t *__restrict__ chunk_len)
{
    const int lane = threadIdx.x & 63;
    const uint32_t x = blockIdx.x * 4 + (threadIdx.x >> 6);
    if (x >= n_long) return;
    const K1Long lg = longs[x];
    const uint32_t g = lg.w / (uint32_t)n_frames;
    const int f = (int)(lg.w % (uint32_t)n_frames) + 1;
    const int64_t L = (int64_t)(off[g + 1] - off[g]);
    const int64_t na = frame_len(L, f);
    const int64_t n_words = (na + 1 + 63) >> 6;
    const unsigned long long *mk = mask + lg.mask_off;
    uint32_t *starts = chunk_off + chunk_base[lg.w];
    constexpr int ROWS = 4, WIN = 64 * ROWS;
    const int n_w = (int)n_words, n_a = (int)na;
    auto load = [&](int base, unsigned long long *dst) {
#pragma unroll
        for (int r = 0; r < ROWS; ++r) dst[r] = mk[min(base + 64 * r + lane, n_w - 1)];
    };
    auto take = [&](int base, const unsigned long long *src, unsigned long long *dst) {
#pragma unroll
        for (int r = 0; r < ROWS; ++r) dst[r] = base + 64 * r + lane < n_w ? src[r] : 0ull;
    };
    unsigned long long cur[ROWS], nxt[ROWS];
    int win = 0;
    load(0, nxt);
    take(0, nxt, cur);
    load(WIN, nxt);
    uint32_t cnt = 0;
    int c0 = 0;
    while (c0 < n_a + 1) {
        if (lane == 0) starts[cnt] = (uint32_t)c0;
        ++cnt;
        int end = n_a;
        if (n_a + 1 - c0 >= 1001) {
            int p = c0 + 1000;
            for (;;) {
                int wi = p >> 6;
                if (wi >= win + 2 * WIN) { win = wi; load(win, nxt); take(win, nxt, cur); load(win + WIN, nxt); }
                else if (wi >= win + WIN) {
                    win += WIN;
                    take(win, nxt, cur);
                    load(win + WIN, nxt);
                }
                const int r0 = (wi - win) >> 6, j = (wi - win) & 63;
                unsigned long long v = r0 == 0 ? cur[0] : r0 == 1 ? cur[1] : r0 == 2 ? cur[2] : cur[3];
                v = lane > j ? v : (lane == j ? v & (~0ull << (p & 63)) : 0ull);
                const unsigned long long any = __ballot(v != 0ull);
                if (any) {
                    const int l = __ffsll((long long)any) - 1;
                    const unsigned long long word = ((unsigned long long)(uint32_t)__builtin_amdgcn_readlane((int)(uint32_t)(v >> 32), l) << 32) | (uint32_t)__builtin_amdgcn_readlane((int)(uint32_t)v, l);
                    end = ((win + 64 * r0 + l) << 6) + (int)__builtin_ctzll(word);
                    break;
                }
                p = (win + 64 * (r0 + 1)) << 6;
            }
        }
        c0 = end + 1;
    }
    __builtin_amdgcn_fence(__ATOMIC_RELEASE, "workgroup");
    __builtin_amdgcn_wave_barrier();
    __builtin_amdgcn_fence(__ATOMIC_ACQUIRE, "workgroup");
    uint32_t *lens = chunk_len + chunk_base[lg.w];
    uint32_t kept = cnt;
    for (uint32_t i = (uint32_t)lane; i < cnt; i += 64) {
        const uint32_t s0 = __builtin_nontemporal_load(&starts[i]);
        lens[i] = i + 1 < cnt ? __builtin_nontemporal_load(&starts[i + 1]) - s0 : (uint32_t)(na - (int64_t)s0);
    }
    if (cnt && (int64_t)__builtin_nontemporal_load(&starts[cnt - 1]) >= na) kept = cnt - 1;
    if (lane == 0) chunk_cnt[lg.w] = kept;
}

__global__ __launch_bounds__(256) void k1_ref_chunks(const uint8_t *__restrict__ nt, const uint64_t *__restrict__ off, uint32_t n, int n_frames, int tab,
                                                     const uint64_t *__restrict__ chunk_base, uint32_t *__restrict__ chunk_cnt,
                                                     uint32_t *__restrict__ chunk_off, uint32_t *__restrict__ chunk_len, int64_t long_from)
{
    const int lane = threadIdx.x & 63;
    const uint64_t w = (uint64_t)blockIdx.x * 4 + (threadIdx.x >> 6);
    if (w >= (uint64_t)n * n_frames) return;
    const uint32_t g = (uint32_t)(w / n_frames);
    const int f = (int)(w % n_frames) + 1;
    const uint8_t *s = nt + off[g];
    const int64_t L = (int64_t)(off[g + 1] - off[g]);
    const int64_t na = frame_len(L, f);
    if (na + 1 > long_from) return;
    const uint64_t base = chunk_base[w];
    uint32_t cnt = 0;
    int64_t c0 = 0;
    while (c0 < na + 1) {
        const int64_t end = chunk_end(s, L, f, tab, na, c0, lane);
        int64_t len = end - c0 + 1;
        if (end == na) --len;
        if (len > 0) {
            if (lane == 0) { chunk_off[base + cnt] = (uint32_t)c0; chunk_len[base + cnt] = (uint32_t)len; }
            ++cnt;
        }
        c0 = end + 1;
    }
    if (lane == 0) chunk_cnt[w] = cnt;
}

__global__ __launch_bounds__(256) void k1_pack(const uint8_t *__restrict__ nt, const K1Src *__restrict__ src_of, int tab,
                                               const PackDesc *__restrict__ desc, const uint32_t *__restrict__ pk_off, const uint32_t *__restrict__ n_ptr, uint32_t cap,
                                               uint8_t *__restrict__ res, uint2 *__restrict__ blk2seq, const K1Summary *__restrict__ d_sum, K1Summary *__restrict__ pin_sum)
{
    const int lane = threadIdx.x & 63;
    const uint32_t s = blockIdx.x * 4 + (threadIdx.x >> 6);
    if (blockIdx.x == 0 && threadIdx.x == 0) *pin_sum = *d_sum;
    const uint32_t n_packed = *n_ptr;
    const uint32_t sc = min(s, cap);
    const PackDesc d = desc[sc];
    const K1Src so = src_of[sc];
    const uint32_t start = pk_off[sc], next = pk_off[sc + 1];
    __shared__ uint32_t codon_all[4][64];
    uint32_t *codon = codon_all[threadIdx.x >> 6];
    codon[lane] = c_codon[tab][lane];
    if (n_packed == 0) {
        if (s == 0) for (uint32_t x = lane; x < pk_off[0]; x += 64) res[x] = (uint8_t)PEP_PAD_CODE;
        return;
    }
    if (s >= n_packed) return;
    const uint8_t *src = nt + so.off;
    const int L = (int)so.L;
    if (s == 0) for (uint32_t x = lane; x < start; x += 64) res[x] = (uint8_t)PEP_PAD_CODE;
    __shared__ uint32_t stage_all[4][392];
    uint32_t *stage = stage_all[threadIdx.x >> 6];
    const int frame = (int)d.frame;
    const bool fwd = frame <= 3;
    const int fo = fwd ? frame - 1 : frame - 4;
    for (uint32_t c0 = 0; c0 < next - start; c0 += 512) {
        const int P0 = fo + 3 * (int)(d.aa_off + c0);
        const int lo = fwd ? P0 : L - 1 - (P0 + 1535);
        int shift = 0;
        if (c0 < d.len && P0 < L) {
            const uintptr_t A = reinterpret_cast<uintptr_t>(src) + (intptr_t)lo;
            shift = (int)(A & 3u);
            const uint32_t *al = reinterpret_cast<const uint32_t *>(A - shift);
            const int first_dw = lo < 0 ? (-lo + shift) >> 2 : 0;
            const int n_dw = (min(1536, L - lo) + shift + 3) >> 2;
            for (int x = first_dw + lane; x < n_dw; x += 64) stage[x] = al[x];
        }
        __builtin_amdgcn_fence(__ATOMIC_RELEASE, "workgroup");
        __builtin_amdgcn_wave_barrier();
        __builtin_amdgcn_fence(__ATOMIC_ACQUIRE, "workgroup");
        const uint32_t x0 = c0 + 8 * lane;
        if (x0 < next - start) {
            const int di = fwd ? 6 * lane : 378 - 6 * lane;
            uint32_t raw[7], ch[6];
#pragma unroll
            for (int k = 0; k < 7; ++k) raw[k] = stage[di + k];
#pragma unroll
            for (int k = 0; k < 6; ++k) ch[k] = __builtin_amdgcn_alignbyte(raw[k + 1], raw[k], (uint32_t)shift);
            if (!fwd) {
#pragma unroll
                for (int k = 0; k < 3; ++k) {
                    const uint32_t lo_w = __builtin_bswap32(ch[5 - k]), hi_w = __builtin_bswap32(ch[k]);
                    ch[k] = lo_w; ch[5 - k] = hi_w;
                }
            }
            const int n_valid = min(max(L - (P0 + 24 * lane), 0), 24);
            const int n_res = (int)min(max((int64_t)d.len - (int64_t)x0, (int64_t)0), (int64_t)8);
            uint32_t word[2];
#pragma unroll
            for (int h = 0; h < 2; ++h) {
                uint32_t pk[3], bad[3];
#pragma unroll
                for (int k = 0; k < 3; ++k) nt4(ch[3 * h + k], !fwd, pk[k], bad[k]);
                const uint32_t codes = (pk[0] << 16) | (pk[1] << 8) | pk[2];
                uint32_t bad12 = (bad[0] << 8) | (bad[1] << 4) | bad[2];
                const int nv = min(max(n_valid - 12 * h, 0), 12);
                bad12 |= (1u << (12 - nv)) - 1u;
                uint32_t w = 0;
#pragma unroll
                for (int k = 0; k < 4; ++k) {
                    uint32_t c = codon[(codes >> (18 - 6 * k)) & 63u];
                    if ((bad12 >> (9 - 3 * k)) & 7u) c = 23u;
                    if (4 * h + k >= n_res) c = PEP_PAD_CODE;
                    w |= c << (8 * k);
                }
                word[h] = w;
            }
            *reinterpret_cast<uint2 *>(res + start + x0) = make_uint2(word[0], word[1]);
        }
        __builtin_amdgcn_wave_barrier();
    }
    for (uint32_t b = (start >> 5) + lane, last = ((next & 31u) == 16u) ? ((next - 16u) >> 5) - 1u : (next - 17u) >> 5; b <= last && last != ~0u; b += 64) blk2seq[b] = make_uint2(s, start);
}

constexpr uint32_t NUCL_SLICE = 32768;
__global__ __launch_bounds__(256) void nucl_pack(const uint8_t *__restrict__ nt, const uint64_t *__restrict__ nt_off, const NuclDesc *__restrict__ desc,
                                                 const uint32_t *__restrict__ pk_off, uint32_t n_packed, uint8_t *__restrict__ res, uint2 *__restrict__ blk2seq)
{
    const int lane = threadIdx.x & 63;
    const uint32_t s = blockIdx.x * 4 + (threadIdx.x >> 6);
    if (n_packed == 0) {
        if (s == 0) for (uint32_t x = lane; x < pk_off[0]; x += 64) res[x] = (uint8_t)PEP_PAD_CODE;
        return;
    }
    if (s >= n_packed) return;
    const NuclDesc d = desc[s];
    const uint32_t start = pk_off[s], next = pk_off[s + 1];
    const uint8_t *src = nt + nt_off[d.seq];
    const int64_t L = (int64_t)(nt_off[d.seq + 1] - nt_off[d.seq]);
    const uint32_t x_lo = blockIdx.y * NUCL_SLICE, x_hi = min(next - start, x_lo + NUCL_SLICE);
    if (x_lo >= next - start) return;
    if (s == 0 && blockIdx.y == 0) for (uint32_t x = lane; x < start; x += 64) res[x] = (uint8_t)PEP_PAD_CODE;
    for (uint32_t x0 = x_lo + 8 * lane; x0 < x_hi; x0 += 512) {
        uint32_t word[2] = {0, 0};
        uint8_t raw[8];
        const bool whole = (int64_t)x0 + 8 <= L;
        if (whole) __builtin_memcpy(raw, d.rev ? src + (L - 8 - x0) : src + x0, 8);
#pragma unroll
        for (int k = 0; k < 8; ++k) {
            uint32_t c = PEP_PAD_CODE;
            if ((int64_t)x0 + k < L) {
                const uint8_t ch = whole ? raw[d.rev ? 7 - k : k] : (d.rev ? src[L - 1 - x0 - k] : src[x0 + k]);
                const int v = base2(ch);
                c = v < 0 ? 4u : (uint32_t)(d.rev ? 3 - v : v);
            }
            word[k >> 2] |= c << (8 * (k & 3));
        }
        *reinterpret_cast<uint2 *>(res + start + x0) = make_uint2(word[0], word[1]);
    }
    for (uint32_t b = ((start + x_lo) >> 5) + lane, last = min(((next & 31u) == 16u) ? ((next - 16u) >> 5) - 1u : (next - 17u) >> 5, (start + x_hi - 1u) >> 5); b <= last && last != ~0u; b += 64)
        blk2seq[b] = make_uint2(s, start);
}

void fill_codon_table(uint8_t tab[2][64])
{
    static const char *aa = "KNKNTTTTRSRSIIMIQHQHPPPPRRRRLLLLEDEDAAAAGGGGVVVVXYXYSSSSXCWCLFLF";
    for (int i = 0; i < 64; ++i) tab[0][i] = tab[1][i] = (uint8_t)(aa[i] - 'A');
    tab[1][56] = (uint8_t)('W' - 'A');
}

int upload_codon_table(pep_ctx *ctx)
{
    if (ctx->codon_ready) return PEP_OK;
    uint8_t tab[2][64];
    fill_codon_table(tab);
    PEP_HIP(ctx, hipMemcpyToSymbol(HIP_SYMBOL(c_codon), tab, sizeof(tab), 0, hipMemcpyHostToDevice));
    ctx->codon_ready = true;
    return PEP_OK;
}

__global__ void k1_query_desc(uint32_t n, const uint32_t *__restrict__ frame, const uint32_t *__restrict__ len, PackDesc *__restrict__ desc,
                              uint32_t *__restrict__ padded, uint32_t *__restrict__ len_out, uint32_t *__restrict__ n_out, K1Summary *__restrict__ sum,
                              uint32_t *__restrict__ pin_len)
{
    const uint32_t i = blockIdx.x * blockDim.x + threadIdx.x;
    if (i == 0) { *n_out = n; sum->residues = 0ull; sum->max_len = 0u; }
    if (i >= n) return;
    desc[i] = PackDesc{i, frame[i], 0u, len[i]};
    padded[i] = padded_len(len[i]);
    len_out[i] = len[i];
    pin_len[i] = len[i];
}

struct K1Scan { uint64_t *state; uint32_t ticket_base; uint64_t epoch; };

__global__ __launch_bounds__(256) void k1_ref_desc(uint64_t nw, int n_frames, const uint64_t *__restrict__ chunk_base, const uint32_t *__restrict__ chunk_cnt,
                                                   const uint32_t *__restrict__ chunk_off, const uint32_t *__restrict__ chunk_len,
                                                   PackDesc *__restrict__ desc, uint32_t *__restrict__ padded, uint32_t *__restrict__ len_out, K1Summary *__restrict__ sum,
                                                   uint32_t *__restrict__ n_targets, K1Scan sc, const uint64_t *__restrict__ nt_off, K1Src *__restrict__ src_of,
                                                   uint32_t *__restrict__ first_t, uint32_t *__restrict__ first_w, uint32_t fill_from)
{
    __shared__ uint32_t s_tile, lds[4];
    __shared__ uint64_t s_pre;
    const uint32_t tile = lb_take_tile(sc.state, sc.ticket_base, &s_tile);
    const uint64_t w = (uint64_t)tile * 256 + threadIdx.x;
    if (w == 0) { sum->residues = 0ull; sum->max_len = 0u; }
    const uint32_t cnt = w < nw ? chunk_cnt[w] : 0u;
    uint32_t tot;
    const uint32_t ex = block_excl_scan_256<uint32_t>(cnt, &tot, lds);
    if (threadIdx.x < 64) {
        const uint64_t p = lb_tile_prefix<32>(sc.state + 1, tile, tot, sc.epoch, (int)threadIdx.x);
        if (threadIdx.x == 0) s_pre = p;
    }
    __syncthreads();
    if (tile == gridDim.x - 1 && threadIdx.x == 255) *n_targets = (uint32_t)(s_pre + tot);
    if (w >= nw) return;
    const uint32_t g = (uint32_t)(w / n_frames), f = (uint32_t)(w % n_frames) + 1;
    const uint64_t base = chunk_base[w];
    const uint32_t at = (uint32_t)s_pre + ex;
    if (f == 1u) first_t[g] = cnt ? at : PEP_SELF_NONE;
    const uint64_t o = nt_off[g];
    const K1Src so{o, (uint32_t)(nt_off[g + 1] - o), 0u};
    first_w[w] = at;
    if (cnt >= fill_from) return;
    for (uint32_t c = 0; c < cnt; ++c) {
        desc[at + c] = PackDesc{g, f, chunk_off[base + c], chunk_len[base + c]};
        src_of[at + c] = so;
        padded[at + c] = padded_len(chunk_len[base + c]);
        len_out[at + c] = chunk_len[base + c];
    }
}

__global__ __launch_bounds__(256) void k1_ref_desc_fill(const K1Seg *__restrict__ tiles, int n_frames, const uint64_t *__restrict__ chunk_base, const uint32_t *__restrict__ chunk_cnt,
                                                        const uint32_t *__restrict__ chunk_off, const uint32_t *__restrict__ chunk_len, const uint32_t *__restrict__ first_w,
                                                        uint32_t fill_from, PackDesc *__restrict__ desc, uint32_t *__restrict__ padded, uint32_t *__restrict__ len_out,
                                                        const uint64_t *__restrict__ nt_off, K1Src *__restrict__ src_of)
{
    const K1Seg tl = tiles[blockIdx.x];
    const uint32_t w = tl.w, c = tl.seg * 256u + threadIdx.x, cnt = chunk_cnt[w];
    if (cnt < fill_from || c >= cnt) return;
    const uint32_t g = w / (uint32_t)n_frames, f = w % (uint32_t)n_frames + 1u;
    const uint64_t base = chunk_base[w], o = nt_off[g];
    const uint32_t at = first_w[w] + c, len = chunk_len[base + c];
    desc[at] = PackDesc{g, f, chunk_off[base + c], len};
    src_of[at] = K1Src{o, (uint32_t)(nt_off[g + 1] - o), 0u};
    padded[at] = padded_len(len);
    len_out[at] = len;
}

__global__ __launch_bounds__(256) void k1_offsets(const uint32_t *__restrict__ n_ptr, const uint32_t *__restrict__ padded, uint32_t cap, uint32_t *__restrict__ pk_off,
                                                  const uint32_t *__restrict__ len, K1Summary *__restrict__ sum, K1Scan sc)
{
    __shared__ uint32_t s_tile, lds[4];
    __shared__ uint64_t s_pre;
    __shared__ unsigned long long blk_s[4];
    __shared__ uint32_t blk_m[4];
    const uint32_t tile = lb_take_tile(sc.state, sc.ticket_base, &s_tile);
    const uint32_t i = tile * 256 + threadIdx.x;
    const uint32_t n = *n_ptr;
    const uint32_t pad = i < n ? padded[i] : 0u;
    uint32_t tot;
    const uint32_t ex = block_excl_scan_256<uint32_t>(pad, &tot, lds);
    if (threadIdx.x < 64) {
        const uint64_t p = lb_tile_prefix<32>(sc.state + 1, tile, tot, sc.epoch, (int)threadIdx.x);
        if (threadIdx.x == 0) s_pre = p;
    }
    __syncthreads();
    const uint32_t at = (uint32_t)s_pre + ex;
    if (i <= cap) pk_off[i] = i < n ? at + PEP_END_PAD : at + 2 * PEP_END_PAD;
    uint32_t L = i < n ? len[i] : 0u, m = L;
    unsigned long long s = L;
    for (int d = 32; d > 0; d >>= 1) { s += __shfl_xor(s, d, 64); m = max(m, (uint32_t)__shfl_xor((int)m, d, 64)); }
    if ((threadIdx.x & 63) == 0) { blk_s[threadIdx.x >> 6] = s; blk_m[threadIdx.x >> 6] = m; }
    __syncthreads();
    if (threadIdx.x == 0) {
        const uint32_t bm = max(max(blk_m[0], blk_m[1]), max(blk_m[2], blk_m[3]));
        if (bm) { atomicAdd(&sum->residues, blk_s[0] + blk_s[1] + blk_s[2] + blk_s[3]); atomicMax(&sum->max_len, bm); }
    }
    if (i == cap) { sum->n = n; sum->total = (unsigned long long)at + 2ull * PEP_END_PAD; }
}

int reserve_packed(pep_ctx *ctx, SeqSet &out, uint32_t cap, uint64_t upper)
{
    if (upper > PEP_MAX_RESIDUES + (uint64_t)cap * 32) return pep_fail(ctx, PEP_ERR_LIMIT, "packed protein set exceeds 2^29 bytes");
    PEP_TRY(dev_reserve(ctx, out.res, upper + 64));
    PEP_TRY(dev_reserve(ctx, out.off, ((size_t)cap + 2) * 4));
    PEP_TRY(dev_reserve(ctx, out.len, ((size_t)cap + 2) * 4));
    PEP_TRY(dev_reserve(ctx, out.blk2seq, (upper / 32 + 2) * sizeof(uint2)));
    return PEP_OK;
}

int layout_and_pack(pep_ctx *ctx, const NtSet &nt, int tab, const PackDesc *d_desc, const uint32_t *d_padded, uint32_t cap, const uint32_t *d_n,
                    uint64_t upper, SeqSet &out, DevBuf &d_scan, DevBuf &tmp, K1Summary *pin_sum)
{
    (void)d_scan; (void)tmp;
    K1Summary *d_sum = reinterpret_cast<K1Summary *>(const_cast<PackDesc *>(d_desc) + cap);
    K1Scan sc;
    const uint64_t tiles = ceil_div((uint64_t)cap + 1, 256);
    PEP_TRY(pep_lookback_begin(ctx, ctx->scan_state[0], tiles, (1u << 30) - 1, &sc.state, &sc.ticket_base, &sc.epoch));
    hipLaunchKernelGGL(k1_offsets, dim3((unsigned)tiles), dim3(256), 0, ctx->stream, d_n, d_padded, cap, out.off.as<uint32_t>(), out.len.as<const uint32_t>(), d_sum, sc);
    hipLaunchKernelGGL(k1_pack, dim3((unsigned)ceil_div((uint64_t)cap + 1, 4)), dim3(256), 0, ctx->stream, nt.nt.as<const uint8_t>(), (const K1Src *)k1_src_of(d_desc, cap), tab,
                       d_desc, out.off.as<const uint32_t>(), d_n, cap, out.res.as<uint8_t>(), out.blk2seq.as<uint2>(), (const K1Summary *)d_sum, pin_sum);
    PEP_HIP(ctx, hipGetLastError());
    return PEP_OK;
}

int take_summary(pep_ctx *ctx, const void *pinned, SeqSet &out)
{
    const K1Summary *sum = reinterpret_cast<const K1Summary *>(pinned);
    if (sum->total > PEP_MAX_RESIDUES) return pep_fail(ctx, PEP_ERR_LIMIT, "packed protein set exceeds 2^29 bytes");
    if (sum->max_len > PEP_MAX_SEQ_LEN) return pep_fail(ctx, PEP_ERR_LIMIT, "protein longer than PEP_MAX_SEQ_LEN");
    out.n = sum->n; out.total = sum->total; out.residues = sum->residues; out.max_len = sum->max_len;
    return PEP_OK;
}

void finish_layout(const PackDesc *desc, uint32_t n, SeqSet &out)
{
    out.h_off.resize((size_t)n + 1);
    out.h_len.resize(n);
    uint64_t pos = PEP_END_PAD;
    for (uint32_t i = 0; i < n; ++i) {
        out.h_off[i] = (uint32_t)pos;
        out.h_len[i] = desc[i].len;
        pos += ((uint64_t)desc[i].len + 15) / 16 * 16 + PEP_SEQ_GAP;
    }
    out.h_off[n] = (uint32_t)(pos + PEP_END_PAD);
}

int k1_ref_finish(pep_ctx *ctx)
{
    PEP_HIP(ctx, pep_event_wait(ctx->k1_event));
    PEP_TRY(take_summary(ctx, ctx->pin_k1.p, ctx->t));
    ctx->t_tables_lazy = true;
    return PEP_OK;
}

}

int pep_k1_query(pep_ctx *ctx, int gtable, int phase)
{
    const NtSet &nt = ctx->q_nt;
    const int tab = gtable == 4 ? 1 : 0;
    const uint32_t n = nt.n;
    if (phase != 2) {
        PEP_TRY(upload_codon_table(ctx));
        if (n > PEP_MAX_QUERIES) return pep_fail(ctx, PEP_ERR_LIMIT, "too many queries");
        DevBuf *W = ctx->ws;
        PEP_TRY(dev_reserve(ctx, W[0], ((size_t)n + 1) * 4));
        PEP_TRY(dev_reserve(ctx, W[1], ((size_t)n + 1) * 4));
        DevBuf &D = ctx->d_k1_desc_q;
        PEP_TRY(dev_reserve(ctx, D, (2 * (size_t)n + 4) * sizeof(PackDesc)));
        PEP_TRY(pin_reserve(ctx, ctx->pin_k1q, sizeof(K1Summary) + ((size_t)n + 1) * 4));
        K1Summary *pin_sum = reinterpret_cast<K1Summary *>(ctx->pin_k1q.p);
        uint32_t *pin_len = reinterpret_cast<uint32_t *>(ctx->pin_k1q.p + sizeof(K1Summary));
        PEP_TRY(dev_reserve(ctx, W[3], ((size_t)n + 1) * 4));
        PEP_TRY(dev_reserve(ctx, W[5], 16));
        const uint64_t upper = 2 * PEP_END_PAD + (nt.total + 2 * (uint64_t)n) / 3 + (uint64_t)n * (16 + PEP_SEQ_GAP);
        PEP_TRY(reserve_packed(ctx, ctx->q, n, upper));
        if (n) hipLaunchKernelGGL(k1_query_frames, dim3((unsigned)ceil_div(n, 4)), dim3(256), 0, ctx->stream, nt.nt.as<const uint8_t>(), nt.off.as<const uint64_t>(), n, tab,
                                  D.as<PackDesc>(), W[3].as<uint32_t>(), ctx->q.len.as<uint32_t>(), W[5].as<uint32_t>(), reinterpret_cast<K1Summary *>(D.as<PackDesc>() + n), pin_len,
                                  k1_src_of(D.as<const PackDesc>(), n));
        else hipLaunchKernelGGL(k1_query_desc, dim3(1), dim3(64), 0, ctx->stream, 0u, (const uint32_t *)nullptr, (const uint32_t *)nullptr,
                                D.as<PackDesc>(), W[3].as<uint32_t>(), ctx->q.len.as<uint32_t>(), W[5].as<uint32_t>(), reinterpret_cast<K1Summary *>(D.as<PackDesc>() + n), pin_len);
        PEP_TRY(layout_and_pack(ctx, nt, tab, D.as<const PackDesc>(), W[3].as<const uint32_t>(), n, W[5].as<const uint32_t>(), upper, ctx->q, W[4], W[6], pin_sum));
        ctx->k1q_event_set = false;
        if (ctx->k1q_event || hipEventCreateWithFlags(&ctx->k1q_event, pep_wait_event_flags()) == hipSuccess)
            ctx->k1q_event_set = hipEventRecord(ctx->k1q_event, ctx->stream) == hipSuccess;
    }
    if (phase == 1) return PEP_OK;
    if (ctx->k1q_event_set) PEP_HIP(ctx, pep_event_wait(ctx->k1q_event));
    else PEP_HIP(ctx, pep_stream_wait(ctx));
    ctx->k1q_event_set = false;
    PEP_TRY(take_summary(ctx, ctx->pin_k1q.p, ctx->q));
    const uint32_t *pin_len = reinterpret_cast<const uint32_t *>(ctx->pin_k1q.p + sizeof(K1Summary));
    ctx->q.h_len.assign(pin_len, pin_len + n);
    ctx->q_tables_lazy = true;
    return PEP_OK;
}

int pep_k1_host_tables(pep_ctx *ctx)
{
    if (ctx->t_tables_lazy) {
        const uint32_t n = ctx->t.n;
        std::vector<PackDesc> fetched((size_t)n + 1);
        if (n) { PEP_TRY(pep_d2h_queue(ctx, fetched.data(), ctx->d_k1_desc_t.p, (size_t)n * sizeof(PackDesc))); PEP_HIP(ctx, pep_stream_wait(ctx)); pep_d2h_finish(ctx); }
        const PackDesc *desc = fetched.data();
        ctx->t_meta.resize(n);
        for (uint32_t i = 0; i < n; ++i) ctx->t_meta[i] = pep_target_meta{desc[i].seq, desc[i].frame, desc[i].aa_off, desc[i].len};
        finish_layout(desc, n, ctx->t);
        ctx->t_tables_lazy = false;
    }
    return pep_k1_host_tables_q(ctx);
}

int pep_k1_host_tables_q(pep_ctx *ctx)
{
    if (ctx->q_tables_lazy) {
        const NtSet &nt = ctx->q_nt;
        const uint32_t n = ctx->q.n;
        std::vector<PackDesc> fetched((size_t)n + 1);
        if (n) { PEP_TRY(pep_d2h_queue(ctx, fetched.data(), ctx->d_k1_desc_q.p, (size_t)n * sizeof(PackDesc))); PEP_HIP(ctx, pep_stream_wait(ctx)); pep_d2h_finish(ctx); }
        const PackDesc *desc = fetched.data();
        ctx->q_meta.resize(n);
        for (uint32_t i = 0; i < n; ++i) ctx->q_meta[i] = pep_query_meta{i, desc[i].frame, desc[i].len, (uint32_t)(nt.h_off[i + 1] - nt.h_off[i])};
        finish_layout(desc, n, ctx->q);
        ctx->q_tables_lazy = false;
    }
    return PEP_OK;
}

int pep_k1_ref(pep_ctx *ctx, int frames, int gtable, int phase)
{
    const NtSet &nt = ctx->r_nt;
    const int tab = gtable == 4 ? 1 : 0;
    if (phase == 2) return k1_ref_finish(ctx);
    PEP_TRY(upload_codon_table(ctx));
    const uint32_t n = nt.n;
    const int nf = frames == 3 ? 3 : 6;
    const uint64_t nw = (uint64_t)n * nf;
    if (ctx->k1_base_frames != nf) {
        std::vector<uint64_t> &base = ctx->k1_base;
        base.assign(nw + 1, 0);
        uint64_t upper = 2 * PEP_END_PAD;
        for (uint32_t g = 0; g < n; ++g) {
            const uint64_t L = nt.h_off[g + 1] - nt.h_off[g];
            for (int f = 1; f <= nf; ++f) {
                const uint64_t shift = (uint64_t)(f <= 3 ? f - 1 : f - 4);
                const uint64_t na = L > shift ? (L - shift + 2) / 3 : 0;
                const uint64_t slots_w = (na + 1) / 1001 + 1;
                base[(uint64_t)g * nf + f] = base[(uint64_t)g * nf + f - 1] + slots_w;
                upper += na + slots_w * (15 + PEP_SEQ_GAP);
            }
        }
        ctx->k1_upper = upper;
        PEP_TRY(dev_reserve(ctx, ctx->d_k1_base, (nw + 1) * 8));
        PEP_HIP(ctx, hipMemcpy(ctx->d_k1_base.p, base.data(), (nw + 1) * 8, hipMemcpyHostToDevice));
        std::vector<K1Seg> segs, tiles;
        std::vector<K1Long> longs;
        std::vector<uint32_t> long_of_w;
        uint64_t mask_words = 0;
        for (uint32_t g = 0; g < n; ++g) {
            const uint64_t L = nt.h_off[g + 1] - nt.h_off[g];
            for (int f = 1; f <= nf; ++f) {
                const uint64_t shift = (uint64_t)(f <= 3 ? f - 1 : f - 4);
                const uint64_t na = L > shift ? (L - shift + 2) / 3 : 0;
                if (na + 1 <= (uint64_t)K1_LONG) continue;
                const uint32_t w = g * (uint32_t)nf + (uint32_t)(f - 1);
                if (long_of_w.empty()) long_of_w.assign(nw, 0u);
                long_of_w[w] = (uint32_t)longs.size();
                longs.push_back(K1Long{w, 0u, mask_words});
                const uint64_t n_words = (na + 1 + 63) / 64;
                mask_words += n_words;
                for (uint32_t k = 0, nt_ = (uint32_t)((n_words + 63) / 64); k < nt_; ++k) segs.push_back(K1Seg{w, k});
                for (uint32_t k = 0, n_tiles = (uint32_t)(((na + 1) / 1001 + 1 + 255) / 256); k < n_tiles; ++k) tiles.push_back(K1Seg{w, k});
            }
        }
        ctx->k1_n_seg = (uint32_t)segs.size();
        ctx->k1_n_long = (uint32_t)longs.size();
        if (!segs.empty()) {
            PEP_TRY(dev_reserve(ctx, ctx->d_k1_seg, segs.size() * sizeof(K1Seg)));
            PEP_TRY(dev_reserve(ctx, ctx->d_k1_long, longs.size() * sizeof(K1Long) + (size_t)nw * 4));
            PEP_TRY(dev_reserve(ctx, ctx->d_k1_spec, (mask_words + 1) * 8));
            PEP_HIP(ctx, hipMemcpy(ctx->d_k1_seg.p, segs.data(), segs.size() * sizeof(K1Seg), hipMemcpyHostToDevice));
            PEP_HIP(ctx, hipMemcpy(ctx->d_k1_long.p, longs.data(), longs.size() * sizeof(K1Long), hipMemcpyHostToDevice));
            PEP_HIP(ctx, hipMemcpy(ctx->d_k1_long.as<char>() + longs.size() * sizeof(K1Long), long_of_w.data(), (size_t)nw * 4, hipMemcpyHostToDevice));
            PEP_TRY(dev_reserve(ctx, ctx->d_k1_tiles, tiles.size() * sizeof(K1Seg)));
            PEP_HIP(ctx, hipMemcpy(ctx->d_k1_tiles.p, tiles.data(), tiles.size() * sizeof(K1Seg), hipMemcpyHostToDevice));
        }
        ctx->k1_n_tiles = (uint32_t)tiles.size();
        ctx->k1_base_frames = nf;
    }
    const uint64_t slots = ctx->k1_base[nw], upper = ctx->k1_upper;
    if (slots > PEP_MAX_TARGETS) return pep_fail(ctx, PEP_ERR_LIMIT, "too many targets");
    DevBuf *W = ctx->ws;
    PEP_TRY(dev_reserve(ctx, W[1], (nw + 1) * 4));
    PEP_TRY(dev_reserve(ctx, W[2], (slots + 1) * 4));
    PEP_TRY(dev_reserve(ctx, W[3], (slots + 1) * 4));
    DevBuf &D = ctx->d_k1_desc_t;
    PEP_TRY(dev_reserve(ctx, D, (2 * slots + 4) * sizeof(PackDesc)));
    PEP_TRY(pin_reserve(ctx, ctx->pin_k1, sizeof(K1Summary)));
    K1Summary *pin_sum = reinterpret_cast<K1Summary *>(ctx->pin_k1.p);
    PEP_TRY(dev_reserve(ctx, W[5], (nw + 2) * 4));
    PEP_TRY(dev_reserve(ctx, W[6], (slots + 1) * 4));
    PEP_TRY(reserve_packed(ctx, ctx->t, (uint32_t)slots, upper));
    PEP_TRY(dev_reserve(ctx, ctx->d_self_t, ((size_t)n + 1) * 4));
    ctx->self_first_n = n;
    const uint64_t *d_base = ctx->d_k1_base.as<const uint64_t>();
    if (nw) {
        hipLaunchKernelGGL(k1_ref_chunks, dim3((unsigned)ceil_div(nw, 4)), dim3(256), 0, ctx->stream, nt.nt.as<const uint8_t>(), nt.off.as<const uint64_t>(), n, nf, tab,
                           d_base, W[1].as<uint32_t>(), W[2].as<uint32_t>(), W[3].as<uint32_t>(), ctx->k1_n_long ? K1_LONG : INT64_MAX);
        if (ctx->k1_n_long) {
            const K1Long *d_longs = ctx->d_k1_long.as<const K1Long>();
            const uint32_t *d_long_of_w = reinterpret_cast<const uint32_t *>(ctx->d_k1_long.as<const char>() + (size_t)ctx->k1_n_long * sizeof(K1Long));
            hipLaunchKernelGGL(k1_stop_mask, dim3((unsigned)ceil_div(ctx->k1_n_seg, 4)), dim3(256), 0, ctx->stream, nt.nt.as<const uint8_t>(), nt.off.as<const uint64_t>(), nf, tab,
                               ctx->d_k1_seg.as<const K1Seg>(), ctx->k1_n_seg, d_longs, d_long_of_w, ctx->d_k1_spec.as<unsigned long long>());
            hipLaunchKernelGGL(k1_ref_chunks_mask, dim3((unsigned)ceil_div(ctx->k1_n_long, 4)), dim3(256), 0, ctx->stream, nt.off.as<const uint64_t>(), nf, d_longs, ctx->k1_n_long,
                               ctx->d_k1_spec.as<const unsigned long long>(), d_base, W[1].as<uint32_t>(), W[2].as<uint32_t>(), W[3].as<uint32_t>());
        }
        {
            K1Scan sc;
            const uint64_t tiles = ceil_div(nw, 256);
            PEP_TRY(pep_lookback_begin(ctx, ctx->scan_state[0], tiles, (1u << 30) - 1, &sc.state, &sc.ticket_base, &sc.epoch));
            hipLaunchKernelGGL(k1_ref_desc, dim3((unsigned)tiles), dim3(256), 0, ctx->stream, nw, nf, d_base, W[1].as<const uint32_t>(),
                               W[2].as<const uint32_t>(), W[3].as<const uint32_t>(), D.as<PackDesc>(), W[6].as<uint32_t>(),
                               ctx->t.len.as<uint32_t>(), reinterpret_cast<K1Summary *>(D.as<PackDesc>() + slots), W[5].as<uint32_t>() + nw, sc,
                               nt.off.as<const uint64_t>(), k1_src_of(D.as<const PackDesc>(), (uint32_t)slots), ctx->d_self_t.as<uint32_t>(), W[5].as<uint32_t>(),
                               ctx->k1_n_tiles ? K1_FILL_FROM : 0xFFFFFFFFu);
            if (ctx->k1_n_tiles)
                hipLaunchKernelGGL(k1_ref_desc_fill, dim3(ctx->k1_n_tiles), dim3(256), 0, ctx->stream, ctx->d_k1_tiles.as<const K1Seg>(), nf, d_base, W[1].as<const uint32_t>(),
                                   W[2].as<const uint32_t>(), W[3].as<const uint32_t>(), W[5].as<const uint32_t>(), K1_FILL_FROM, D.as<PackDesc>(), W[6].as<uint32_t>(),
                                   ctx->t.len.as<uint32_t>(), nt.off.as<const uint64_t>(), k1_src_of(D.as<const PackDesc>(), (uint32_t)slots));
        }
        PEP_TRY(layout_and_pack(ctx, nt, tab, D.as<const PackDesc>(), W[6].as<const uint32_t>(), (uint32_t)slots, W[5].as<const uint32_t>() + nw, upper, ctx->t,
                                W[7], W[8], pin_sum));
    } else {
        PEP_HIP(ctx, hipMemsetAsync(W[5].p, 0, 8, ctx->stream));
        PEP_HIP(ctx, hipMemsetAsync(W[6].p, 0, 4, ctx->stream));
        PEP_HIP(ctx, hipMemsetAsync(D.p, 0, 3 * sizeof(PackDesc), ctx->stream));
        PEP_TRY(layout_and_pack(ctx, nt, tab, D.as<const PackDesc>(), W[6].as<const uint32_t>(), 0, W[5].as<const uint32_t>(), upper, ctx->t, W[7], W[8], pin_sum));
    }
    ctx->k1_desc_cap = (uint32_t)slots;
    if (!ctx->k1_event && hipEventCreateWithFlags(&ctx->k1_event, pep_wait_event_flags()) != hipSuccess) return pep_fail(ctx, PEP_ERR_HIP, "hipEventCreate failed");
    PEP_HIP(ctx, hipEventRecord(ctx->k1_event, ctx->stream));
    if (phase == 1) return PEP_OK;
    return k1_ref_finish(ctx);
}

int pep_self_map(pep_ctx *ctx, int *on)
{
    *on = 0;
    const SeqSet &Q = ctx->q, &T = ctx->t;
    if (!ctx->q_from_nt || !ctx->t_from_nt || Q.n == 0 || T.n == 0) return PEP_OK;
    if (ctx->resid_from_nucl) {
        if (!ctx->nucl_valid || !ctx->nucl_t.d_first.p || ctx->nucl_t.n_first == 0) return PEP_OK;
        ctx->self_first = ctx->nucl_t.d_first.as<const uint32_t>(); ctx->self_first_cnt = ctx->nucl_t.n_first; ctx->self_exact_len = 1;
    } else {
        if (!ctx->d_self_t.p || ctx->self_first_n == 0) return PEP_OK;
        ctx->self_first = ctx->d_self_t.as<const uint32_t>(); ctx->self_first_cnt = ctx->self_first_n; ctx->self_exact_len = 0;
    }
    if (ctx->self_first_cnt != Q.n) return PEP_OK;
    const size_t blocks = (size_t)(T.total / 32 + 16);
    PEP_TRY(dev_reserve(ctx, ctx->d_self_delta, blocks * 4));
    PEP_HIP(ctx, hipMemsetAsync(ctx->d_self_delta.p, 0x80, blocks * 4, ctx->stream));
    *on = 1;
    return PEP_OK;
}

static int nucl_build(pep_ctx *ctx, const NtSet &nt, const std::vector<NuclDesc> &order, uint32_t max_n, SeqSet &out, pep_ctx::NuclSide &keep)
{
    const uint32_t n = (uint32_t)order.size();
    if (n > max_n) return pep_fail(ctx, PEP_ERR_LIMIT, "too many sequences");
    keep.h_off.assign((size_t)n + 1, 0);
    keep.h_len.assign(n, 0);
    uint64_t pos = PEP_END_PAD, residues = 0;
    uint32_t max_len = 0;
    for (uint32_t i = 0; i < n; ++i) {
        const uint64_t len = nt.h_off[order[i].seq + 1] - nt.h_off[order[i].seq];
        if (len > PEP_MAX_SEQ_LEN) return pep_fail(ctx, PEP_ERR_LIMIT, "sequence longer than PEP_MAX_SEQ_LEN");
        keep.h_off[i] = (uint32_t)pos; keep.h_len[i] = (uint32_t)len;
        residues += len; max_len = std::max(max_len, (uint32_t)len);
        pos += (len + 15) / 16 * 16 + PEP_SEQ_GAP;
        if (pos > PEP_MAX_RESIDUES) return pep_fail(ctx, PEP_ERR_LIMIT, "packed sequence set exceeds 2^29 bytes");
    }
    pos += PEP_END_PAD;
    keep.h_off[n] = (uint32_t)pos;
    keep.n = n; keep.total = pos; keep.residues = residues; keep.max_len = max_len;
    PEP_TRY(dev_reserve(ctx, keep.d_off, ((size_t)n + 2) * 4));
    PEP_TRY(dev_reserve(ctx, keep.d_len, ((size_t)n + 2) * 4));
    PEP_TRY(dev_reserve(ctx, keep.d_desc, ((size_t)n + 1) * sizeof(NuclDesc)));
    PEP_HIP(ctx, hipMemcpyAsync(keep.d_off.p, keep.h_off.data(), ((size_t)n + 1) * 4, hipMemcpyHostToDevice, ctx->stream));
    if (n) PEP_HIP(ctx, hipMemcpyAsync(keep.d_len.p, keep.h_len.data(), (size_t)n * 4, hipMemcpyHostToDevice, ctx->stream));
    if (n) PEP_HIP(ctx, hipMemcpyAsync(keep.d_desc.p, order.data(), (size_t)n * sizeof(NuclDesc), hipMemcpyHostToDevice, ctx->stream));
    PEP_HIP(ctx, hipStreamSynchronize(ctx->stream));
    (void)out;
    return PEP_OK;
}

static int nucl_apply(pep_ctx *ctx, const NtSet &nt, const pep_ctx::NuclSide &keep, SeqSet &out)
{
    const uint32_t n = keep.n;
    out.n = n; out.total = keep.total; out.residues = keep.residues; out.max_len = keep.max_len;
    out.h_off = keep.h_off; out.h_len = keep.h_len;
    PEP_TRY(dev_reserve(ctx, out.res, keep.total + 64));
    PEP_TRY(dev_reserve(ctx, out.off, ((size_t)n + 2) * 4));
    PEP_TRY(dev_reserve(ctx, out.len, ((size_t)n + 2) * 4));
    PEP_TRY(dev_reserve(ctx, out.blk2seq, (keep.total / 32 + 2) * sizeof(uint2)));
    PEP_HIP(ctx, hipMemcpyAsync(out.off.p, keep.d_off.p, ((size_t)n + 1) * 4, hipMemcpyDeviceToDevice, ctx->stream));
    if (n) PEP_HIP(ctx, hipMemcpyAsync(out.len.p, keep.d_len.p, (size_t)n * 4, hipMemcpyDeviceToDevice, ctx->stream));
    hipLaunchKernelGGL(nucl_pack, dim3((unsigned)ceil_div((uint64_t)n + 1, 4), (unsigned)ceil_div((uint64_t)keep.max_len + 15 + PEP_SEQ_GAP, NUCL_SLICE) + 1), dim3(256), 0, ctx->stream, nt.nt.as<const uint8_t>(), nt.off.as<const uint64_t>(),
                       keep.d_desc.as<const NuclDesc>(), out.off.as<const uint32_t>(), n, out.res.as<uint8_t>(), out.blk2seq.as<uint2>());
    PEP_HIP(ctx, hipGetLastError());
    return PEP_OK;
}

int pep_nucl_sets(pep_ctx *ctx, int strands)
{
    if (!ctx->nucl_valid || ctx->nucl_strands != strands) {
        ctx->nucl_valid = false;
        std::vector<NuclDesc> qo(ctx->q_nt.n), to;
        for (uint32_t i = 0; i < ctx->q_nt.n; ++i) qo[i] = NuclDesc{i, 0u};
        PEP_TRY(nucl_build(ctx, ctx->q_nt, qo, PEP_MAX_QUERIES, ctx->q, ctx->nucl_q));
        const uint32_t nr = ctx->r_nt.n;
        const bool grouped = ctx->group_of_seq.size() == nr && nr > 0;
        to.reserve((size_t)nr * strands);
        for (uint32_t a = 0; a < nr;) {
            uint32_t b = a + 1;
            while (b < nr && (!grouped || ctx->group_of_seq[b] == ctx->group_of_seq[a])) ++b;
            for (int rev = 0; rev < strands; ++rev)
                for (uint32_t i = a; i < b; ++i) to.push_back(NuclDesc{i, (uint32_t)rev});
            a = b;
        }
        PEP_TRY(nucl_build(ctx, ctx->r_nt, to, PEP_MAX_TARGETS, ctx->t, ctx->nucl_t));
        {
            std::vector<uint32_t> first(nr, PEP_SELF_NONE);
            for (size_t i = 0; i < to.size(); ++i) if (!to[i].rev) first[to[i].seq] = (uint32_t)i;
            PEP_TRY(dev_reserve(ctx, ctx->nucl_t.d_first, ((size_t)nr + 1) * 4));
            if (nr) PEP_HIP(ctx, hipMemcpy(ctx->nucl_t.d_first.p, first.data(), (size_t)nr * 4, hipMemcpyHostToDevice));
            ctx->nucl_t.n_first = nr;
        }
        ctx->nucl_q.q_meta.resize(ctx->q_nt.n);
        for (uint32_t i = 0; i < ctx->q_nt.n; ++i) ctx->nucl_q.q_meta[i] = pep_query_meta{i, 1u, ctx->nucl_q.h_len[i], ctx->nucl_q.h_len[i]};
        ctx->nucl_t.t_meta.resize(to.size());
        for (size_t i = 0; i < to.size(); ++i) ctx->nucl_t.t_meta[i] = pep_target_meta{to[i].seq, to[i].rev ? 4u : 1u, 0u, ctx->nucl_t.h_len[i]};
        ctx->nucl_strands = strands;
        ctx->nucl_valid = true;
    }
    PEP_TRY(nucl_apply(ctx, ctx->q_nt, ctx->nucl_q, ctx->q));
    PEP_TRY(nucl_apply(ctx, ctx->r_nt, ctx->nucl_t, ctx->t));
    ctx->q_tables_lazy = false;
    ctx->t_tables_lazy = false;
    ctx->q_meta = ctx->nucl_q.q_meta;
    ctx->t_meta = ctx->nucl_t.t_meta;
    return PEP_OK;
}
```

Measured before the change: 24.22 million gene-pairs/s.

## Run reference k1 translation on a side stream concurrent with query k1

Forks a second HIP stream so the reference-side k1 translation/pack kernels run concurrently with the query-side k1 work, joining before targets are used. To make the overlap safe, the reference path gets its own workspace buffers and lookback scan state. This adds stream/event management and extra device memory, and it risks races if any shared buffer was missed.

After: 24.07 million gene-pairs/s, median of 2. About the same (-0.6%).

```diff
diff --git a/peppan_amd/csrc/capi.hip b/peppan_amd/csrc/capi.hip
--- a/peppan_amd/csrc/capi.hip
+++ b/peppan_amd/csrc/capi.hip
@@ -15,6 +15,7 @@
         ctx->pin_small_used = 0;
         for (auto &st : ctx->fused_state) st.dirty = true;
         for (auto &st : ctx->scan_state) st.dirty = true;
+        ctx->k1r_scan.dirty = true;
         ctx->sort_dirty = true;
         ctx->zero_clean = false;
         for (bool &f : ctx->zero_ok) f = false;
@@ -213,6 +214,27 @@
     const hipError_t r = hipEventRecord(ctx->wait_event, ctx->stream);
     if (r != hipSuccess) return hipStreamSynchronize(ctx->stream);
     return pep_event_wait(ctx->wait_event);
+}
+
+int pep_side_fork(pep_ctx *ctx)
+{
+    PEP_HIP(ctx, hipEventRecord(ctx->fork_event, ctx->stream));
+    PEP_HIP(ctx, hipStreamWaitEvent(ctx->side, ctx->fork_event, 0));
+    ctx->side_busy = true;
+    return PEP_OK;
+}
+
+int pep_side_join(pep_ctx *ctx)
+{
+    if (!ctx->side_busy) return PEP_OK;
+    ctx->side_busy = false;
+    hipError_t e = hipEventRecord(ctx->join_event, ctx->side);
+    if (e == hipSuccess) e = hipStreamWaitEvent(ctx->stream, ctx->join_event, 0);
+    if (e != hipSuccess) {
+        (void)hipStreamSynchronize(ctx->side);
+        return pep_fail(ctx, PEP_ERR_HIP, std::string("side stream join: ") + hipGetErrorString(e));
+    }
+    return PEP_OK;
 }
 
 int pep_sync_reads(pep_ctx *ctx)
@@ -485,6 +507,8 @@
     pep_default_params(&ctx->params);
     if (hipSetDevice(device) != hipSuccess) { delete ctx; return PEP_ERR_HIP; }
     if (hipStreamCreate(&ctx->stream) != hipSuccess) { delete ctx; return PEP_ERR_HIP; }
+    if (hipStreamCreate(&ctx->side) != hipSuccess || hipEventCreateWithFlags(&ctx->fork_event, hipEventDisableTiming) != hipSuccess ||
+        hipEventCreateWithFlags(&ctx->join_event, hipEventDisableTiming) != hipSuccess) { pep_ctx_destroy(ctx); return PEP_ERR_HIP; }
     if (pin_reserve(ctx, ctx->pin_small, 16384) != PEP_OK) { *out = ctx; return PEP_ERR_HIP; }
     int rc = pep_selftest_dpp(ctx);
     if (rc != PEP_OK) { *out = ctx; return rc; }
@@ -496,7 +520,10 @@
 {
     if (!ctx) return;
     (void)hipSetDevice(ctx->device);
+    if (ctx->side) (void)hipStreamSynchronize(ctx->side);
+    if (ctx->stream) (void)hipStreamSynchronize(ctx->stream);
     for (auto &b : ctx->ws) dev_release(b);
+    for (auto &b : ctx->k1r_ws) dev_release(b);
     for (int id = 0; id < TM_COUNT; ++id) { if (ctx->tm_a[id]) (void)hipEventDestroy(ctx->tm_a[id]); if (ctx->tm_b[id]) (void)hipEventDestroy(ctx->tm_b[id]); }
     pep_drop_dev_result(ctx);
     if (ctx->staged_result) {
@@ -517,11 +544,14 @@
     if (ctx->pin_down.p) (void)hipHostFree(ctx->pin_down.p);
     if (ctx->pin_up.p) (void)hipHostFree(ctx->pin_up.p);
     if (ctx->pin_ms.p) (void)hipHostFree(ctx->pin_ms.p);
-    DevBuf *bufs[] = {&ctx->sub_lds, &ctx->d_params, &ctx->scan_state[0].buf, &ctx->scan_state[1].buf, &ctx->fused_state[0].buf, &ctx->fused_state[1].buf, &ctx->fused_state[2].buf, &ctx->fused_state[3].buf, &ctx->d_min_score, &ctx->d_trace_mode, &ctx->d_trace_defer, &ctx->d_k1_base, &ctx->d_k1_seg, &ctx->d_k1_long, &ctx->d_k1_spec, &ctx->d_k1_tiles, &ctx->d_t_class, &ctx->d_t_subject, &ctx->d_nt_match, &ctx->q_nt.nt, &ctx->q_nt.off, &ctx->r_nt.nt, &ctx->r_nt.off,
+    DevBuf *bufs[] = {&ctx->sub_lds, &ctx->d_params, &ctx->scan_state[0].buf, &ctx->scan_state[1].buf, &ctx->k1r_scan.buf, &ctx->fused_state[0].buf, &ctx->fused_state[1].buf, &ctx->fused_state[2].buf, &ctx->fused_state[3].buf, &ctx->d_min_score, &ctx->d_trace_mode, &ctx->d_trace_defer, &ctx->d_k1_base, &ctx->d_k1_seg, &ctx->d_k1_long, &ctx->d_k1_spec, &ctx->d_k1_tiles, &ctx->d_t_class, &ctx->d_t_subject, &ctx->d_nt_match, &ctx->q_nt.nt, &ctx->q_nt.off, &ctx->r_nt.nt, &ctx->r_nt.off,
                       &ctx->q.res, &ctx->q.off, &ctx->q.len, &ctx->t.res, &ctx->t.off, &ctx->t.len, &ctx->q.blk2seq, &ctx->t.blk2seq,
                       &ctx->sort_state, &ctx->sort_hist, &ctx->d_set, &ctx->d_zero, &ctx->d_k1_desc_q, &ctx->d_k1_desc_t, &ctx->d_self_delta, &ctx->d_self_t, &ctx->d_mail_copy,
                       &ctx->nucl_q.d_off, &ctx->nucl_q.d_len, &ctx->nucl_q.d_desc, &ctx->nucl_t.d_off, &ctx->nucl_t.d_len, &ctx->nucl_t.d_desc, &ctx->nucl_t.d_first};
     for (DevBuf *b : bufs) dev_release(*b);
+    if (ctx->fork_event) (void)hipEventDestroy(ctx->fork_event);
+    if (ctx->join_event) (void)hipEventDestroy(ctx->join_event);
+    if (ctx->side) (void)hipStreamDestroy(ctx->side);
     if (ctx->stream) (void)hipStreamDestroy(ctx->stream);
     delete ctx;
 }
@@ -705,6 +735,7 @@
     if (!ctx || !out) return PEP_ERR_ARG;
     *out = nullptr;
     PEP_HIP(ctx, hipSetDevice(ctx->device));
+    SideJoinGuard side_guard(ctx);
     pep_materialise_staged(ctx);
     if (params) {
         if (params->n_shapes < 1 || params->n_shapes > 4 || params->base < 2 || params->top_k < 1 || params->n_splits < 1)
@@ -738,8 +769,11 @@
     if (!ctx->resid_from_nucl) {
         const bool do_q = ctx->q_from_nt && !ctx->q_ready, do_t = ctx->t_from_nt && !ctx->t_ready;
         if ((do_q || do_t) && ctx->timing_level < 2 && ctx->group_of_seq.empty()) {
+            if (do_t) {
+                PEP_TRY(pep_side_fork(ctx));
+                PEP_TRY(pep_k1_ref(ctx, ctx->t_frames, ctx->t_gtable, 1, ctx->side));
+            }
             if (do_q) PEP_TRY(pep_k1_query(ctx, ctx->q_gtable, 1));
-            if (do_t) PEP_TRY(pep_k1_ref(ctx, ctx->t_frames, ctx->t_gtable, 1));
             if (do_q) { PEP_TRY(pep_k1_query(ctx, ctx->q_gtable, 2)); ctx->q_ready = true; }
             ctx->k1_t_deferred = do_t;
             ctx->stats.ms_k1 = 0.;
@@ -750,6 +784,7 @@
         if (!c->k1_t_deferred) return PEP_OK;
         c->k1_t_deferred = false;
         PEP_TRY(pep_k1_ref(c, c->t_frames, c->t_gtable, 2));
+        PEP_TRY(pep_side_join(c));
         c->t_ready = true;
         c->stats.target_residues = c->t.residues;
         return PEP_OK;
@@ -800,6 +835,7 @@
     if (counted)
         rc = ctx->ext.pending ? pep_k7_hits_queue(ctx, ctx->ext.n_bound, reinterpret_cast<const pep_hit *>(ctx->ext.d_hits), reinterpret_cast<const uint32_t *>(ctx->ext.d_cig), ctx->ext.d_n_hits)
                               : pep_k7_hits_queue(ctx, res->n_hits, res->d_hits, res->d_cigar);
+    { const int jrc = pep_side_join(ctx); if (rc == PEP_OK) rc = jrc; }
     pep_timer_end(ctx, TM_TOTAL);
     const hipError_t se = pep_stream_wait(ctx);
     if (rc == PEP_OK && se != hipSuccess) rc = pep_fail(ctx, PEP_ERR_HIP, std::string("stream sync: ") + hipGetErrorString(se));
diff --git a/peppan_amd/csrc/common.h b/peppan_amd/csrc/common.h
--- a/peppan_amd/csrc/common.h
+++ b/peppan_amd/csrc/common.h
@@ -70,6 +70,9 @@
 struct pep_ctx {
     int device = 0;
     hipStream_t stream = nullptr;
+    hipStream_t side = nullptr;
+    hipEvent_t fork_event = nullptr, join_event = nullptr;
+    bool side_busy = false;
     PinBuf pin_small;
     size_t pin_small_used = 0;
     struct PendingRead { void *dst; size_t off, n; } pending[32];
@@ -116,6 +119,7 @@
     int k1_base_frames = 0;
     DevBuf d_k1_seg, d_k1_long, d_k1_spec, d_k1_tiles;
     uint32_t k1_n_seg = 0, k1_n_long = 0, k1_n_tiles = 0;
+    DevBuf k1r_ws[5];
     struct NuclSide {
         uint32_t n = 0, max_len = 0;
         uint64_t total = 0, residues = 0;
@@ -148,6 +152,7 @@
     struct ScanState { DevBuf buf; uint32_t epoch = 0, ticket_base = 0; bool dirty = false; };
     ScanState fused_state[4];
     ScanState scan_state[2];
+    ScanState k1r_scan;
     DevBuf sort_state, sort_hist;
     uint32_t sort_epoch = 0, sort_ticket_base = 0;
     bool sort_dirty = false;
@@ -222,6 +227,16 @@
 int pep_sync_reads(pep_ctx *ctx);
 hipError_t pep_stream_wait(pep_ctx *ctx);
 hipError_t pep_event_wait(hipEvent_t ev);
+int pep_side_fork(pep_ctx *ctx);
+int pep_side_join(pep_ctx *ctx);
+static inline bool pep_side_on(const pep_ctx *ctx) { return ctx->timing_level < 2 && ctx->side != nullptr; }
+struct SideJoinGuard {
+    pep_ctx *ctx;
+    explicit SideJoinGuard(pep_ctx *c) : ctx(c) {}
+    ~SideJoinGuard() { if (ctx->side_busy) (void)pep_side_join(ctx); }
+    SideJoinGuard(const SideJoinGuard &) = delete;
+    SideJoinGuard &operator=(const SideJoinGuard &) = delete;
+};
 int pin_reserve(pep_ctx *ctx, PinBuf &b, size_t bytes);
 int pep_h2d(pep_ctx *ctx, void *d_dst, const void *h_src, size_t n);
 int pep_d2h_queue(pep_ctx *ctx, void *h_dst, const void *d_src, size_t n);
@@ -257,7 +272,7 @@
                  const pep_key_unpack *unpack);
 int pep_sort_u64_two_level(pep_ctx *ctx, uint64_t *d_keys, uint64_t *d_tmp, uint64_t n, int bits, const uint32_t *d_top_hist, const pep_key_unpack *unpack);
 int pep_k1_query(pep_ctx *ctx, int gtable, int phase = 0);
-int pep_k1_ref(pep_ctx *ctx, int frames, int gtable, int phase = 0);
+int pep_k1_ref(pep_ctx *ctx, int frames, int gtable, int phase = 0, hipStream_t st = nullptr);
 int pep_k1_host_tables(pep_ctx *ctx);
 int pep_k1_host_tables_q(pep_ctx *ctx);
 int pep_nucl_sets(pep_ctx *ctx, int strands);
diff --git a/peppan_amd/csrc/lookback.h b/peppan_amd/csrc/lookback.h
--- a/peppan_amd/csrc/lookback.h
+++ b/peppan_amd/csrc/lookback.h
@@ -52,4 +52,5 @@
     return base + inc - v;
 }
 
-int pep_lookback_begin(pep_ctx *ctx, pep_ctx::ScanState &S, uint64_t n_tiles, uint32_t epoch_mask, uint64_t **state, uint32_t *ticket_base, uint64_t *epoch);
+int pep_lookback_begin(pep_ctx *ctx, pep_ctx::ScanState &S, uint64_t n_tiles, uint32_t epoch_mask, uint64_t **state, uint32_t *ticket_base, uint64_t *epoch,
+                       hipStream_t st = nullptr);
diff --git a/peppan_amd/csrc/scan.hip b/peppan_amd/csrc/scan.hip
--- a/peppan_amd/csrc/scan.hip
+++ b/peppan_amd/csrc/scan.hip
@@ -245,7 +245,7 @@
     return PEP_OK;
 }
 
-int pep_lookback_begin(pep_ctx *ctx, pep_ctx::ScanState &S, uint64_t n_tiles, uint32_t epoch_mask, uint64_t **state, uint32_t *ticket_base, uint64_t *epoch)
+int pep_lookback_begin(pep_ctx *ctx, pep_ctx::ScanState &S, uint64_t n_tiles, uint32_t epoch_mask, uint64_t **state, uint32_t *ticket_base, uint64_t *epoch, hipStream_t st)
 {
     bool clear = false;
     if ((n_tiles + 1) * sizeof(uint64_t) > S.buf.cap) {
@@ -256,7 +256,7 @@
     S.epoch = (S.epoch + 1) & epoch_mask;
     if (S.epoch == 0) { clear = true; S.epoch = 1; }
     if (clear) {
-        PEP_HIP(ctx, hipMemsetAsync(S.buf.p, 0, S.buf.cap, ctx->stream));
+        PEP_HIP(ctx, hipMemsetAsync(S.buf.p, 0, S.buf.cap, st ? st : ctx->stream));
         S.ticket_base = 0;
     }
     *state = S.buf.as<uint64_t>();
diff --git a/peppan_amd/csrc/translate.hip b/peppan_amd/csrc/translate.hip
--- a/peppan_amd/csrc/translate.hip
+++ b/peppan_amd/csrc/translate.hip
@@ -567,15 +567,14 @@
 }
 
 int layout_and_pack(pep_ctx *ctx, const NtSet &nt, int tab, const PackDesc *d_desc, const uint32_t *d_padded, uint32_t cap, const uint32_t *d_n,
-                    uint64_t upper, SeqSet &out, DevBuf &d_scan, DevBuf &tmp, K1Summary *pin_sum)
-{
-    (void)d_scan; (void)tmp;
+                    uint64_t upper, SeqSet &out, hipStream_t st, pep_ctx::ScanState &scan, K1Summary *pin_sum)
+{
     K1Summary *d_sum = reinterpret_cast<K1Summary *>(const_cast<PackDesc *>(d_desc) + cap);
     K1Scan sc;
     const uint64_t tiles = ceil_div((uint64_t)cap + 1, 256);
-    PEP_TRY(pep_lookback_begin(ctx, ctx->scan_state[0], tiles, (1u << 30) - 1, &sc.state, &sc.ticket_base, &sc.epoch));
-    hipLaunchKernelGGL(k1_offsets, dim3((unsigned)tiles), dim3(256), 0, ctx->stream, d_n, d_padded, cap, out.off.as<uint32_t>(), out.len.as<const uint32_t>(), d_sum, sc);
-    hipLaunchKernelGGL(k1_pack, dim3((unsigned)ceil_div((uint64_t)cap + 1, 4)), dim3(256), 0, ctx->stream, nt.nt.as<const uint8_t>(), (const K1Src *)k1_src_of(d_desc, cap), tab,
+    PEP_TRY(pep_lookback_begin(ctx, scan, tiles, (1u << 30) - 1, &sc.state, &sc.ticket_base, &sc.epoch, st));
+    hipLaunchKernelGGL(k1_offsets, dim3((unsigned)tiles), dim3(256), 0, st, d_n, d_padded, cap, out.off.as<uint32_t>(), out.len.as<const uint32_t>(), d_sum, sc);
+    hipLaunchKernelGGL(k1_pack, dim3((unsigned)ceil_div((uint64_t)cap + 1, 4)), dim3(256), 0, st, nt.nt.as<const uint8_t>(), (const K1Src *)k1_src_of(d_desc, cap), tab,
                        d_desc, out.off.as<const uint32_t>(), d_n, cap, out.res.as<uint8_t>(), out.blk2seq.as<uint2>(), (const K1Summary *)d_sum, pin_sum);
     PEP_HIP(ctx, hipGetLastError());
     return PEP_OK;
@@ -638,7 +637,7 @@
                                   k1_src_of(D.as<const PackDesc>(), n));
         else hipLaunchKernelGGL(k1_query_desc, dim3(1), dim3(64), 0, ctx->stream, 0u, (const uint32_t *)nullptr, (const uint32_t *)nullptr,
                                 D.as<PackDesc>(), W[3].as<uint32_t>(), ctx->q.len.as<uint32_t>(), W[5].as<uint32_t>(), reinterpret_cast<K1Summary *>(D.as<PackDesc>() + n), pin_len);
-        PEP_TRY(layout_and_pack(ctx, nt, tab, D.as<const PackDesc>(), W[3].as<const uint32_t>(), n, W[5].as<const uint32_t>(), upper, ctx->q, W[4], W[6], pin_sum));
+        PEP_TRY(layout_and_pack(ctx, nt, tab, D.as<const PackDesc>(), W[3].as<const uint32_t>(), n, W[5].as<const uint32_t>(), upper, ctx->q, ctx->stream, ctx->scan_state[0], pin_sum));
         ctx->k1q_event_set = false;
         if (ctx->k1q_event || hipEventCreateWithFlags(&ctx->k1q_event, pep_wait_event_flags()) == hipSuccess)
             ctx->k1q_event_set = hipEventRecord(ctx->k1q_event, ctx->stream) == hipSuccess;
@@ -685,8 +684,9 @@
     return PEP_OK;
 }
 
-int pep_k1_ref(pep_ctx *ctx, int frames, int gtable, int phase)
-{
+int pep_k1_ref(pep_ctx *ctx, int frames, int gtable, int phase, hipStream_t st)
+{
+    if (!st) st = ctx->stream;
     const NtSet &nt = ctx->r_nt;
     const int tab = gtable == 4 ? 1 : 0;
     if (phase == 2) return k1_ref_finish(ctx);
@@ -748,56 +748,56 @@
     }
     const uint64_t slots = ctx->k1_base[nw], upper = ctx->k1_upper;
     if (slots > PEP_MAX_TARGETS) return pep_fail(ctx, PEP_ERR_LIMIT, "too many targets");
-    DevBuf *W = ctx->ws;
-    PEP_TRY(dev_reserve(ctx, W[1], (nw + 1) * 4));
+    DevBuf *W = ctx->k1r_ws;
+    PEP_TRY(dev_reserve(ctx, W[0], (nw + 1) * 4));
+    PEP_TRY(dev_reserve(ctx, W[1], (slots + 1) * 4));
     PEP_TRY(dev_reserve(ctx, W[2], (slots + 1) * 4));
-    PEP_TRY(dev_reserve(ctx, W[3], (slots + 1) * 4));
     DevBuf &D = ctx->d_k1_desc_t;
     PEP_TRY(dev_reserve(ctx, D, (2 * slots + 4) * sizeof(PackDesc)));
     PEP_TRY(pin_reserve(ctx, ctx->pin_k1, sizeof(K1Summary)));
     K1Summary *pin_sum = reinterpret_cast<K1Summary *>(ctx->pin_k1.p);
-    PEP_TRY(dev_reserve(ctx, W[5], (nw + 2) * 4));
-    PEP_TRY(dev_reserve(ctx, W[6], (slots + 1) * 4));
+    PEP_TRY(dev_reserve(ctx, W[3], (nw + 2) * 4));
+    PEP_TRY(dev_reserve(ctx, W[4], (slots + 1) * 4));
     PEP_TRY(reserve_packed(ctx, ctx->t, (uint32_t)slots, upper));
     PEP_TRY(dev_reserve(ctx, ctx->d_self_t, ((size_t)n + 1) * 4));
     ctx->self_first_n = n;
     const uint64_t *d_base = ctx->d_k1_base.as<const uint64_t>();
     if (nw) {
-        hipLaunchKernelGGL(k1_ref_chunks, dim3((unsigned)ceil_div(nw, 4)), dim3(256), 0, ctx->stream, nt.nt.as<const uint8_t>(), nt.off.as<const uint64_t>(), n, nf, tab,
-                           d_base, W[1].as<uint32_t>(), W[2].as<uint32_t>(), W[3].as<uint32_t>(), ctx->k1_n_long ? K1_LONG : INT64_MAX);
+        hipLaunchKernelGGL(k1_ref_chunks, dim3((unsigned)ceil_div(nw, 4)), dim3(256), 0, st, nt.nt.as<const uint8_t>(), nt.off.as<const uint64_t>(), n, nf, tab,
+                           d_base, W[0].as<uint32_t>(), W[1].as<uint32_t>(), W[2].as<uint32_t>(), ctx->k1_n_long ? K1_LONG : INT64_MAX);
         if (ctx->k1_n_long) {
             const K1Long *d_longs = ctx->d_k1_long.as<const K1Long>();
             const uint32_t *d_long_of_w = reinterpret_cast<const uint32_t *>(ctx->d_k1_long.as<const char>() + (size_t)ctx->k1_n_long * sizeof(K1Long));
-            hipLaunchKernelGGL(k1_stop_mask, dim3((unsigned)ceil_div(ctx->k1_n_seg, 4)), dim3(256), 0, ctx->stream, nt.nt.as<const uint8_t>(), nt.off.as<const uint64_t>(), nf, tab,
+            hipLaunchKernelGGL(k1_stop_mask, dim3((unsigned)ceil_div(ctx->k1_n_seg, 4)), dim3(256), 0, st, nt.nt.as<const uint8_t>(), nt.off.as<const uint64_t>(), nf, tab,
                                ctx->d_k1_seg.as<const K1Seg>(), ctx->k1_n_seg, d_longs, d_long_of_w, ctx->d_k1_spec.as<unsigned long long>());
-            hipLaunchKernelGGL(k1_ref_chunks_mask, dim3((unsigned)ceil_div(ctx->k1_n_long, 4)), dim3(256), 0, ctx->stream, nt.off.as<const uint64_t>(), nf, d_longs, ctx->k1_n_long,
-                               ctx->d_k1_spec.as<const unsigned long long>(), d_base, W[1].as<uint32_t>(), W[2].as<uint32_t>(), W[3].as<uint32_t>());
+            hipLaunchKernelGGL(k1_ref_chunks_mask, dim3((unsigned)ceil_div(ctx->k1_n_long, 4)), dim3(256), 0, st, nt.off.as<const uint64_t>(), nf, d_longs, ctx->k1_n_long,
+                               ctx->d_k1_spec.as<const unsigned long long>(), d_base, W[0].as<uint32_t>(), W[1].as<uint32_t>(), W[2].as<uint32_t>());
         }
         {
             K1Scan sc;
             const uint64_t tiles = ceil_div(nw, 256);
-            PEP_TRY(pep_lookback_begin(ctx, ctx->scan_state[0], tiles, (1u << 30) - 1, &sc.state, &sc.ticket_base, &sc.epoch));
-            hipLaunchKernelGGL(k1_ref_desc, dim3((unsigned)tiles), dim3(256), 0, ctx->stream, nw, nf, d_base, W[1].as<const uint32_t>(),
-                               W[2].as<const uint32_t>(), W[3].as<const uint32_t>(), D.as<PackDesc>(), W[6].as<uint32_t>(),
-                               ctx->t.len.as<uint32_t>(), reinterpret_cast<K1Summary *>(D.as<PackDesc>() + slots), W[5].as<uint32_t>() + nw, sc,
-                               nt.off.as<const uint64_t>(), k1_src_of(D.as<const PackDesc>(), (uint32_t)slots), ctx->d_self_t.as<uint32_t>(), W[5].as<uint32_t>(),
+            PEP_TRY(pep_lookback_begin(ctx, ctx->k1r_scan, tiles, (1u << 30) - 1, &sc.state, &sc.ticket_base, &sc.epoch, st));
+            hipLaunchKernelGGL(k1_ref_desc, dim3((unsigned)tiles), dim3(256), 0, st, nw, nf, d_base, W[0].as<const uint32_t>(),
+                               W[1].as<const uint32_t>(), W[2].as<const uint32_t>(), D.as<PackDesc>(), W[4].as<uint32_t>(),
+                               ctx->t.len.as<uint32_t>(), reinterpret_cast<K1Summary *>(D.as<PackDesc>() + slots), W[3].as<uint32_t>() + nw, sc,
+                               nt.off.as<const uint64_t>(), k1_src_of(D.as<const PackDesc>(), (uint32_t)slots), ctx->d_self_t.as<uint32_t>(), W[3].as<uint32_t>(),
                                ctx->k1_n_tiles ? K1_FILL_FROM : 0xFFFFFFFFu);
             if (ctx->k1_n_tiles)
-                hipLaunchKernelGGL(k1_ref_desc_fill, dim3(ctx->k1_n_tiles), dim3(256), 0, ctx->stream, ctx->d_k1_tiles.as<const K1Seg>(), nf, d_base, W[1].as<const uint32_t>(),
-                                   W[2].as<const uint32_t>(), W[3].as<const uint32_t>(), W[5].as<const uint32_t>(), K1_FILL_FROM, D.as<PackDesc>(), W[6].as<uint32_t>(),
+                hipLaunchKernelGGL(k1_ref_desc_fill, dim3(ctx->k1_n_tiles), dim3(256), 0, st, ctx->d_k1_tiles.as<const K1Seg>(), nf, d_base, W[0].as<const uint32_t>(),
+                                   W[1].as<const uint32_t>(), W[2].as<const uint32_t>(), W[3].as<const uint32_t>(), K1_FILL_FROM, D.as<PackDesc>(), W[4].as<uint32_t>(),
                                    ctx->t.len.as<uint32_t>(), nt.off.as<const uint64_t>(), k1_src_of(D.as<const PackDesc>(), (uint32_t)slots));
         }
-        PEP_TRY(layout_and_pack(ctx, nt, tab, D.as<const PackDesc>(), W[6].as<const uint32_t>(), (uint32_t)slots, W[5].as<const uint32_t>() + nw, upper, ctx->t,
-                                W[7], W[8], pin_sum));
+        PEP_TRY(layout_and_pack(ctx, nt, tab, D.as<const PackDesc>(), W[4].as<const uint32_t>(), (uint32_t)slots, W[3].as<const uint32_t>() + nw, upper, ctx->t,
+                                st, ctx->k1r_scan, pin_sum));
     } else {
-        PEP_HIP(ctx, hipMemsetAsync(W[5].p, 0, 8, ctx->stream));
-        PEP_HIP(ctx, hipMemsetAsync(W[6].p, 0, 4, ctx->stream));
-        PEP_HIP(ctx, hipMemsetAsync(D.p, 0, 3 * sizeof(PackDesc), ctx->stream));
-        PEP_TRY(layout_and_pack(ctx, nt, tab, D.as<const PackDesc>(), W[6].as<const uint32_t>(), 0, W[5].as<const uint32_t>(), upper, ctx->t, W[7], W[8], pin_sum));
+        PEP_HIP(ctx, hipMemsetAsync(W[3].p, 0, 8, st));
+        PEP_HIP(ctx, hipMemsetAsync(W[4].p, 0, 4, st));
+        PEP_HIP(ctx, hipMemsetAsync(D.p, 0, 3 * sizeof(PackDesc), st));
+        PEP_TRY(layout_and_pack(ctx, nt, tab, D.as<const PackDesc>(), W[4].as<const uint32_t>(), 0, W[3].as<const uint32_t>(), upper, ctx->t, st, ctx->k1r_scan, pin_sum));
     }
     ctx->k1_desc_cap = (uint32_t)slots;
     if (!ctx->k1_event && hipEventCreateWithFlags(&ctx->k1_event, pep_wait_event_flags()) != hipSuccess) return pep_fail(ctx, PEP_ERR_HIP, "hipEventCreate failed");
-    PEP_HIP(ctx, hipEventRecord(ctx->k1_event, ctx->stream));
+    PEP_HIP(ctx, hipEventRecord(ctx->k1_event, st));
     if (phase == 1) return PEP_OK;
     return k1_ref_finish(ctx);
 }
```
